# multi-template-matching/MultiTemplateMatching-Python

Hardware: AMD Instinct MI355X
Metric: Mpixel-correlations/s (higher is better)
Workload: dtype u8

## Files before the change

include/mtm_hip.h:

```cpp
#ifndef MTM_HIP_H
#define MTM_HIP_H

#include <stddef.h>
#include <stdint.h>

#ifdef __cplusplus
extern "C" {
#endif

#define MTM_ABI_VERSION 9

#define MTM_U8  0
#define MTM_F32 1
#define MTM_U16 2

#define MTM_TM_SQDIFF        0
#define MTM_TM_SQDIFF_NORMED 1
#define MTM_TM_CCORR         2
#define MTM_TM_CCORR_NORMED  3
#define MTM_TM_CCOEFF        4
#define MTM_TM_CCOEFF_NORMED 5

#define MTM_PEAKS_LOCAL  0
#define MTM_PEAKS_GLOBAL 1
// ... 5 lines not shown
#define MTM_KERNEL_NAIVE 1
#define MTM_KERNEL_DOT4  2
#define MTM_KERNEL_MFMA  3
#define MTM_KERNEL_MFMA16 4

#define MTM_KERNEL_MFMA_F32 5

#define MTM_OPT_KERNEL      1
#define MTM_OPT_PEAK_BORDER 2
#define MTM_OPT_HIT_CAPACITY 3
#define MTM_OPT_DOT4_VARIANT 4
#define MTM_OPT_EXACT_DIV 5
#define MTM_OPT_HITS_ONLY 6
#define MTM_OPT_F32_MFMA 7
#define MTM_OPT_BATCH_MAX_ROWS 8
#define MTM_OPT_BOXES_MAX_FLOATS 9

#define MTM_OK            0
#define MTM_E_INVALID    -1
#define MTM_E_HIP        -2
#define MTM_E_NO_DEVICE  -3
#define MTM_E_STATE      -4
#define MTM_E_OVERFLOW   -5
#define MTM_E_COMM       -6

typedef struct mtm_ctx mtm_ctx;

typedef struct mtm_templ {
    const void* px;
    const void* mask;
    int32_t rows, cols, chans, dtype;
    int64_t row_stride;
    int64_t mask_row_stride;
} mtm_templ;

typedef struct mtm_hit {
    int32_t templ_idx;
    int32_t x, y, w, h;
    float   score;
} mtm_hit;

typedef struct mtm_box_unit {
    int32_t templ_idx;
    int32_t y0, x0, rows, cols;
} mtm_box_unit;

typedef struct mtm_point {
    int32_t templ_idx, x, y;
} mtm_point;

typedef struct mtm_timing {
    float total_ms;
    float score_ms;
    float peaks_ms;
    float ncc_kernel_ms;
    int32_t ncc_launches;
    int32_t kernel_used;
    int64_t n_hits;
    int32_t hits_only;
    float   sclk_mhz;
    float   ncc_sum_ms;
    int32_t f32_route;
    int32_t sq_launches;
    float   masked_stat_ms;
    int32_t f32_pieces;
} mtm_timing;

int         mtm_abi_version(void);
int         mtm_device_count(void);
const char* mtm_last_error(void);
int         mtm_ctx_create(mtm_ctx** out, int device_id);
void        mtm_ctx_destroy(mtm_ctx* ctx);
int         mtm_set_option(mtm_ctx* ctx, int option, int64_t value);
int         mtm_get_option(mtm_ctx* ctx, int option, int64_t* value);
#define MTM_POISON_SCRATCH 1
#define MTM_POISON_LDS     2
#define MTM_POISON_ARENAS  4
int         mtm_debug_poison(mtm_ctx* ctx, int pattern_byte, int what);
int         mtm_debug_quotient_check(mtm_ctx* ctx, uint64_t n_cases, uint64_t seed, uint64_t* out4);
int         mtm_debug_tail_split(int h, int w, double thr);
int         mtm_debug_templ_stats(const void* px, int rows, int cols, int chans, int dtype, int method, double* out7);
#define MTM_CLASS_TILING_FIELDS 12
int         mtm_debug_class_tilings(mtm_ctx* ctx, int32_t* out, int cap_classes);
int         mtm_debug_device_nms(mtm_ctx* ctx, const mtm_hit* hits, int64_t n, int rows, int cols, int max_side,
                                 double score_threshold, int ascending, double max_overlap, int64_t n_min, int64_t n_max,
                                 mtm_hit* out, int64_t capacity, int64_t* n_champions, int64_t* n_undecided);
#define MTM_PEAK_SCAN           0
#define MTM_PEAK_SCAN_BATCH     1
#define MTM_PEAK_SEGMENTS       2
#define MTM_PEAK_VERIFY_MAPS    3
#define MTM_PEAK_VERIFY_HASH    4
#define MTM_PEAK_EXTREMUM       5
#define MTM_PEAK_EXTREMUM_BATCH 6
typedef struct mtm_peak_pass {
    int32_t        n_maps, route, mode_min, border;
    float          thr, thr_q;
    int32_t        img_rows, holes, pattern_byte, reserved;
    int64_t        hit_cap;
    const int32_t* dims;
    const float*   maps;
    const uint8_t* flags;
    const mtm_hit* cands;
    int64_t        n_cands, cand_count, cand_cap;
    mtm_hit*       records;
    int64_t        capacity;
    uint64_t*      count;
    int32_t*       raw;
    int32_t*       trivial;
    int64_t        n_ints;
    uint64_t*      keys;
    mtm_hit*       ext_hits;
    uint64_t*      list_counts;
    int64_t        list_cap;
    int64_t*       info;
} mtm_peak_pass;
int         mtm_debug_peak_pass(mtm_ctx* ctx, const mtm_peak_pass* args);
#define MTM_STATS_FORMS 2
typedef struct mtm_window_stats {
    int32_t        rows, cols, h, w, num_type, form;
    int32_t        tail_s, sb0, sb1, lay_r0, lay_r1, pattern_byte, zero_header, reserved;
    const uint8_t* image;
    double*        t0;
    double*        sum2;
    double*        sq;
    double*        rsq;
    double*        blk;
    double*        blkq;
    uint8_t*       u8;
    uint8_t*       u8b;
    uint64_t*      header;
    int64_t*       info;
} mtm_window_stats;
int         mtm_debug_window_stats(mtm_ctx* ctx, const mtm_window_stats* args);
void*       mtm_host_alloc(size_t bytes);
void        mtm_host_free(void* p);

int mtm_set_image(mtm_ctx* ctx, const void* px, int rows, int cols, int chans, int dtype,
                  int64_t row_stride_bytes);
int mtm_set_image_downscaled(mtm_ctx* ctx, const void* px, int rows, int cols, int chans, int dtype,
                             int64_t row_stride_bytes, int factor);

int mtm_set_templates(mtm_ctx* ctx, const mtm_templ* templs, int n_templ, int method);

typedef struct mtm_variant {
    int32_t rot90;
    int32_t flip_lr;
    int32_t flip_ud;
    int32_t rows, cols;
    int32_t down;
} mtm_variant;
int mtm_set_templates_augmented(mtm_ctx* ctx, const mtm_templ* bases, int n_bases,
                                const mtm_variant* variants, int n_variants, int method);

int mtm_score_map(mtm_ctx* ctx, int templ_idx, float* out, int64_t out_row_stride_bytes);

int mtm_find_matches(mtm_ctx* ctx, int mode, double score_threshold,
                     mtm_hit* out, int64_t capacity, int64_t* n_out);

int mtm_find_matches_image(mtm_ctx* ctx, const void* px, int rows, int cols, int chans, int dtype,
                           int64_t row_stride_bytes, int mode, double score_threshold,
                           mtm_hit* out, int64_t capacity, int64_t* n_out);

int mtm_find_matches_image_nms(mtm_ctx* ctx, const void* px, int rows, int cols, int chans, int dtype,
                               int64_t row_stride_bytes, double score_threshold, double max_overlap, int64_t n_object,
                               mtm_hit* out, int64_t capacity, int64_t* n_out);

// ... 114 lines not shown
```

multitemplatematching-python_amd/MTM/_lib.py:

```python
import ctypes
import struct
import os
import threading
import weakref

import numpy as np

_HERE = os.path.dirname(os.path.abspath(__file__))
LIB_PATH = os.environ.get("MTM_LIB_PATH") or os.path.join(_HERE, "libmtm_hip.so")

MTM_U8, MTM_F32, MTM_U16 = 0, 1, 2
GROUP_EXCHANGE_HOST, GROUP_EXCHANGE_RCCL = 0, 1
PEAKS_LOCAL, PEAKS_GLOBAL = 0, 1
BORDER_CONSTANT, BORDER_NEAREST = 0, 1
KERNEL_AUTO, KERNEL_NAIVE, KERNEL_DOT4, KERNEL_MFMA = 0, 1, 2, 3
OPT_KERNEL, OPT_PEAK_BORDER, OPT_HIT_CAPACITY, OPT_DOT4_VARIANT, OPT_EXACT_DIV, OPT_HITS_ONLY, OPT_F32_MFMA = 1, 2, 3, 4, 5, 6, 7
OPT_BATCH_MAX_ROWS = 8
OPT_BOXES_MAX_FLOATS = 9
ALL_OPTIONS = (OPT_KERNEL, OPT_PEAK_BORDER, OPT_HIT_CAPACITY, OPT_DOT4_VARIANT, OPT_EXACT_DIV, OPT_HITS_ONLY, OPT_F32_MFMA,
               OPT_BATCH_MAX_ROWS, OPT_BOXES_MAX_FLOATS)
BATCH_MAX_ROWS = 65535
POISON_SCRATCH, POISON_LDS, POISON_ARENAS = 1, 2, 4
E_OVERFLOW = -5
E_HIP = -2
COMM_ID_BYTES = 128
ABI_VERSION = 9


class MtmTempl(ctypes.Structure):
    _fields_ = [("px", ctypes.c_void_p), ("mask", ctypes.c_void_p),
                ("rows", ctypes.c_int32), ("cols", ctypes.c_int32),
                ("chans", ctypes.c_int32), ("dtype", ctypes.c_int32),
                ("row_stride", ctypes.c_int64), ("mask_row_stride", ctypes.c_int64)]


class MtmHit(ctypes.Structure):
    _fields_ = [("templ_idx", ctypes.c_int32), ("x", ctypes.c_int32), ("y", ctypes.c_int32),
                ("w", ctypes.c_int32), ("h", ctypes.c_int32), ("score", ctypes.c_float)]


class MtmTiming(ctypes.Structure):
    _fields_ = [("total_ms", ctypes.c_float), ("score_ms", ctypes.c_float),
                ("peaks_ms", ctypes.c_float), ("ncc_kernel_ms", ctypes.c_float),
                ("ncc_launches", ctypes.c_int32), ("kernel_used", ctypes.c_int32),
                ("n_hits", ctypes.c_int64), ("hits_only", ctypes.c_int32), ("sclk_mhz", ctypes.c_float),
                ("ncc_sum_ms", ctypes.c_float), ("f32_route", ctypes.c_int32),
                ("sq_launches", ctypes.c_int32), ("masked_stat_ms", ctypes.c_float),
                ("f32_pieces", ctypes.c_int32)]


HIT_DTYPE = np.dtype([("templ_idx", "<i4"), ("x", "<i4"), ("y", "<i4"), ("w", "<i4"), ("h", "<i4"),
                      ("score", "<f4")])
BOX_UNIT_DTYPE = np.dtype([("templ_idx", "<i4"), ("y0", "<i4"), ("x0", "<i4"), ("rows", "<i4"), ("cols", "<i4")])
BLOCK_DTYPE = np.dtype([("x", "<i4"), ("y", "<i4"), ("w", "<i4"), ("h", "<i4")])
POINT_DTYPE = np.dtype([("templ_idx", "<i4"), ("x", "<i4"), ("y", "<i4")])
assert HIT_DTYPE.itemsize == ctypes.sizeof(MtmHit) == 24
TEMPL_DTYPE = np.dtype([("px", "<u8"), ("mask", "<u8"), ("rows", "<i4"), ("cols", "<i4"), ("chans", "<i4"),
                        ("dtype", "<i4"), ("row_stride", "<i8"), ("mask_row_stride", "<i8")])
assert TEMPL_DTYPE.itemsize == ctypes.sizeof(MtmTempl) == 48
VARIANT_DTYPE = np.dtype([("rot90", "<i4"), ("flip_lr", "<i4"), ("flip_ud", "<i4"), ("rows", "<i4"), ("cols", "<i4"),
                          ("down", "<i4")])

PEAK_SCAN, PEAK_SCAN_BATCH, PEAK_SEGMENTS, PEAK_VERIFY_MAPS, PEAK_VERIFY_HASH, PEAK_EXTREMUM, PEAK_EXTREMUM_BATCH = range(7)
PEAK_INFO_FIELDS = ("grid_x", "grid_y", "grid_z", "list_cap", "n_lists", "verify_blocks", "hash_slots", "extremum_blocks")


class MtmPeakPass(ctypes.Structure):
    _fields_ = [("n_maps", ctypes.c_int32), ("route", ctypes.c_int32), ("mode_min", ctypes.c_int32), ("border", ctypes.c_int32),
                ("thr", ctypes.c_float), ("thr_q", ctypes.c_float),
                ("img_rows", ctypes.c_int32), ("holes", ctypes.c_int32), ("pattern_byte", ctypes.c_int32), ("reserved", ctypes.c_int32),
                ("hit_cap", ctypes.c_int64),
                ("dims", ctypes.c_void_p), ("maps", ctypes.c_void_p), ("flags", ctypes.c_void_p), ("cands", ctypes.c_void_p),
                ("n_cands", ctypes.c_int64), ("cand_count", ctypes.c_int64), ("cand_cap", ctypes.c_int64),
                ("records", ctypes.c_void_p), ("capacity", ctypes.c_int64), ("count", ctypes.c_void_p),
                ("raw", ctypes.c_void_p), ("trivial", ctypes.c_void_p), ("n_ints", ctypes.c_int64),
                ("keys", ctypes.c_void_p), ("ext_hits", ctypes.c_void_p), ("list_counts", ctypes.c_void_p),
                ("list_cap", ctypes.c_int64), ("info", ctypes.c_void_p)]


STATS_FORMS = (8, 4)
STATS_INFO_FIELDS = ("st_pitch", "blk_pitch", "pitch", "form", "grid_x", "grid_y", "n_cus", "kernel_ns")


class MtmWindowStats(ctypes.Structure):
    _fields_ = [("rows", ctypes.c_int32), ("cols", ctypes.c_int32), ("h", ctypes.c_int32), ("w", ctypes.c_int32),
                ("num_type", ctypes.c_int32), ("form", ctypes.c_int32),
                ("tail_s", ctypes.c_int32), ("sb0", ctypes.c_int32), ("sb1", ctypes.c_int32), ("lay_r0", ctypes.c_int32),
                ("lay_r1", ctypes.c_int32), ("pattern_byte", ctypes.c_int32), ("zero_header", ctypes.c_int32),
                ("reserved", ctypes.c_int32),
                ("image", ctypes.c_void_p), ("t0", ctypes.c_void_p), ("sum2", ctypes.c_void_p), ("sq", ctypes.c_void_p),
                ("rsq", ctypes.c_void_p), ("blk", ctypes.c_void_p), ("blkq", ctypes.c_void_p), ("u8", ctypes.c_void_p),
                ("u8b", ctypes.c_void_p), ("header", ctypes.c_void_p), ("info", ctypes.c_void_p)]


_P = ctypes.POINTER
SYMBOLS = {
    "mtm_abi_version": (ctypes.c_int, []),
    "mtm_device_count": (ctypes.c_int, []),
    "mtm_last_error": (ctypes.c_char_p, []),
    "mtm_ctx_create": (ctypes.c_int, [_P(ctypes.c_void_p), ctypes.c_int]),
    "mtm_ctx_destroy": (None, [ctypes.c_void_p]),
    "mtm_set_option": (ctypes.c_int, [ctypes.c_void_p, ctypes.c_int, ctypes.c_int64]),
    "mtm_get_option": (ctypes.c_int, [ctypes.c_void_p, ctypes.c_int, _P(ctypes.c_int64)]),
    "mtm_debug_poison": (ctypes.c_int, [ctypes.c_void_p, ctypes.c_int, ctypes.c_int]),
    "mtm_debug_quotient_check": (ctypes.c_int, [ctypes.c_void_p, ctypes.c_uint64, ctypes.c_uint64, _P(ctypes.c_uint64)]),
    "mtm_debug_tail_split": (ctypes.c_int, [ctypes.c_int, ctypes.c_int, ctypes.c_double]),
    "mtm_debug_class_tilings": (ctypes.c_int, [ctypes.c_void_p, _P(ctypes.c_int32), ctypes.c_int]),
    "mtm_debug_templ_stats": (ctypes.c_int, [ctypes.c_void_p, ctypes.c_int, ctypes.c_int, ctypes.c_int, ctypes.c_int,
                                             ctypes.c_int, _P(ctypes.c_double)]),
    "mtm_debug_device_nms": (ctypes.c_int, [ctypes.c_void_p, ctypes.c_void_p, ctypes.c_int64, ctypes.c_int, ctypes.c_int,
                                            ctypes.c_int, ctypes.c_double, ctypes.c_int, ctypes.c_double, ctypes.c_int64,
                                            ctypes.c_int64, ctypes.c_void_p, ctypes.c_int64, _P(ctypes.c_int64),
                                            _P(ctypes.c_int64)]),
    "mtm_debug_peak_pass": (ctypes.c_int, [ctypes.c_void_p, ctypes.c_void_p]),
    "mtm_debug_window_stats": (ctypes.c_int, [ctypes.c_void_p, ctypes.c_void_p]),
    "mtm_set_image": (ctypes.c_int, [ctypes.c_void_p, ctypes.c_void_p, ctypes.c_int, ctypes.c_int,
                                     ctypes.c_int, ctypes.c_int, ctypes.c_int64]),
    "mtm_set_image_downscaled": (ctypes.c_int, [ctypes.c_void_p, ctypes.c_void_p, ctypes.c_int, ctypes.c_int, ctypes.c_int,
                                                ctypes.c_int, ctypes.c_int64, ctypes.c_int]),
    "mtm_set_templates": (ctypes.c_int, [ctypes.c_void_p, ctypes.c_void_p, ctypes.c_int, ctypes.c_int]),
    "mtm_set_templates_augmented": (ctypes.c_int, [ctypes.c_void_p, ctypes.c_void_p, ctypes.c_int, ctypes.c_void_p, ctypes.c_int,
                                                   ctypes.c_int]),
    "mtm_score_map": (ctypes.c_int, [ctypes.c_void_p, ctypes.c_int, ctypes.c_void_p, ctypes.c_int64]),
    "mtm_find_matches": (ctypes.c_int, [ctypes.c_void_p, ctypes.c_int, ctypes.c_double, ctypes.c_void_p,
                                        ctypes.c_int64, _P(ctypes.c_int64)]),
    "mtm_find_matches_image": (ctypes.c_int, [ctypes.c_void_p, ctypes.c_void_p, ctypes.c_int, ctypes.c_int, ctypes.c_int,
                                              ctypes.c_int, ctypes.c_int64, ctypes.c_int, ctypes.c_double, ctypes.c_void_p,
                                              ctypes.c_int64, _P(ctypes.c_int64)]),
    "mtm_find_matches_image_nms": (ctypes.c_int, [ctypes.c_void_p, ctypes.c_void_p, ctypes.c_int, ctypes.c_int, ctypes.c_int,
                                                  ctypes.c_int, ctypes.c_int64, ctypes.c_double, ctypes.c_double, ctypes.c_int64,
                                                  ctypes.c_void_p, ctypes.c_int64, _P(ctypes.c_int64)]),
    "mtm_find_matches_image_sharded_nms": (ctypes.c_int, [ctypes.c_void_p, ctypes.c_void_p, ctypes.c_int, ctypes.c_int, ctypes.c_int,
                                                          ctypes.c_int, ctypes.c_int64, ctypes.c_double, ctypes.c_double,
                                                          ctypes.c_int64, ctypes.c_int, ctypes.c_void_p, ctypes.c_int,
                                                          ctypes.c_void_p, ctypes.c_int64, _P(ctypes.c_int64)]),
    "mtm_find_matches_batch": (ctypes.c_int, [ctypes.c_void_p, ctypes.c_void_p, ctypes.c_int, ctypes.c_int, ctypes.c_int,
                                              ctypes.c_int, ctypes.c_int, ctypes.c_int64, ctypes.c_int, ctypes.c_double,
                                              ctypes.c_void_p, ctypes.c_int64, ctypes.c_void_p, _P(ctypes.c_int64)]),
    "mtm_find_matches_pyramid": (ctypes.c_int, [ctypes.c_void_p, ctypes.c_void_p, ctypes.c_int, ctypes.c_int, ctypes.c_int,
                                                ctypes.c_int, ctypes.c_int64, ctypes.c_int, ctypes.c_int, ctypes.c_double,
                                                ctypes.c_double, ctypes.c_int, ctypes.c_int, ctypes.c_void_p, ctypes.c_int64,
                                                _P(ctypes.c_int64)]),
    "mtm_find_matches_boxes": (ctypes.c_int, [ctypes.c_void_p, ctypes.c_void_p, ctypes.c_int, ctypes.c_int, ctypes.c_int,
                                              ctypes.c_int, ctypes.c_int64, ctypes.c_void_p, ctypes.c_int, ctypes.c_int,
                                              ctypes.c_double, ctypes.c_void_p, ctypes.c_int64, ctypes.c_void_p,
                                              _P(ctypes.c_int64)]),
    "mtm_track_boxes": (ctypes.c_int, [ctypes.c_void_p, ctypes.c_void_p, ctypes.c_int, ctypes.c_int, ctypes.c_int,
                                       ctypes.c_int, ctypes.c_int, ctypes.c_int64, ctypes.c_void_p, ctypes.c_int, ctypes.c_int,
                                       ctypes.c_int, ctypes.c_double, ctypes.c_void_p]),
    "mtm_track_boxes_nbhd": (ctypes.c_int, [ctypes.c_void_p, ctypes.c_void_p, ctypes.c_int, ctypes.c_int, ctypes.c_int,
                                            ctypes.c_int, ctypes.c_int, ctypes.c_int64, ctypes.c_void_p, ctypes.c_int,
                                            ctypes.c_int, ctypes.c_int, ctypes.c_double, ctypes.c_void_p, ctypes.c_void_p]),
    "mtm_track_boxes_adapt": (ctypes.c_int, [ctypes.c_void_p, ctypes.c_void_p, ctypes.c_int, ctypes.c_int, ctypes.c_int,
                                             ctypes.c_int, ctypes.c_int, ctypes.c_int64, ctypes.c_void_p, ctypes.c_int,
                                             ctypes.c_int, ctypes.c_int, ctypes.c_double, ctypes.c_void_p, ctypes.c_void_p,
                                             ctypes.c_int, ctypes.c_void_p, ctypes.c_void_p]),
    "mtm_track_boxes_reacquire": (ctypes.c_int, [ctypes.c_void_p, ctypes.c_void_p, ctypes.c_int, ctypes.c_int, ctypes.c_int,
                                                 ctypes.c_int, ctypes.c_int, ctypes.c_int64, ctypes.c_void_p, ctypes.c_int,
                                                 ctypes.c_int, ctypes.c_int, ctypes.c_double, ctypes.c_void_p,
                                                 ctypes.c_void_p, ctypes.c_int, ctypes.c_void_p, ctypes.c_void_p]),
    "mtm_track_boxes_sets": (ctypes.c_int, [ctypes.c_void_p, ctypes.c_void_p, ctypes.c_int, ctypes.c_int, ctypes.c_int,
                                            ctypes.c_int, ctypes.c_int, ctypes.c_int64, ctypes.c_void_p, ctypes.c_int,
                                            ctypes.c_void_p, ctypes.c_void_p, ctypes.c_int, ctypes.c_int, ctypes.c_double,
                                            ctypes.c_int, ctypes.c_void_p, ctypes.c_void_p]),
    "mtm_match_blocks": (ctypes.c_int, [ctypes.c_void_p, ctypes.c_void_p, ctypes.c_int64, ctypes.c_void_p, ctypes.c_int64,
                                        ctypes.c_int, ctypes.c_int, ctypes.c_int, ctypes.c_int, ctypes.c_void_p, ctypes.c_int,
                                        ctypes.c_int, ctypes.c_int, ctypes.c_void_p, ctypes.c_void_p]),
    "mtm_debug_plan_blocks": (ctypes.c_int, [ctypes.c_int, ctypes.c_int, ctypes.c_int, ctypes.c_int, ctypes.c_void_p,
                                             ctypes.c_int, ctypes.c_int, ctypes.c_int64, ctypes.c_void_p, ctypes.c_int64,
                                             _P(ctypes.c_int64), ctypes.c_void_p, ctypes.c_void_p, ctypes.c_void_p]),
    "mtm_hit_neighbourhoods": (ctypes.c_int, [ctypes.c_void_p, ctypes.c_void_p, ctypes.c_int, ctypes.c_int, ctypes.c_int,
                                              ctypes.c_int, ctypes.c_int64, ctypes.c_void_p, ctypes.c_int, ctypes.c_void_p]),
    "mtm_find_matches_next": (ctypes.c_int, [ctypes.c_void_p, ctypes.c_int, ctypes.c_double, ctypes.c_void_p,
                                             ctypes.c_int64, _P(ctypes.c_int64), ctypes.c_void_p, ctypes.c_int,
                                             ctypes.c_int, ctypes.c_int, ctypes.c_int, ctypes.c_int64]),
    "mtm_find_matches_async": (ctypes.c_int, [ctypes.c_void_p, ctypes.c_int, ctypes.c_double]),
    "mtm_find_matches_wait": (ctypes.c_int, [ctypes.c_void_p, ctypes.c_void_p, ctypes.c_int64, ctypes.POINTER(ctypes.c_int64)]),
    "mtm_last_hits": (ctypes.c_int, [ctypes.c_void_p, ctypes.c_void_p, ctypes.c_int64, _P(ctypes.c_int64)]),
    "mtm_last_score_map": (ctypes.c_int, [ctypes.c_void_p, ctypes.c_int, ctypes.c_void_p, ctypes.c_int64]),
    "mtm_get_timing": (ctypes.c_int, [ctypes.c_void_p, _P(MtmTiming)]),
    "mtm_nms": (ctypes.c_int, [ctypes.c_void_p, ctypes.c_int64, ctypes.c_double, ctypes.c_int,
                               ctypes.c_int64, ctypes.c_double, ctypes.c_void_p, _P(ctypes.c_int64)]),
    "mtm_nms_segments": (ctypes.c_int, [ctypes.c_void_p, ctypes.c_void_p, ctypes.c_int64, ctypes.c_double, ctypes.c_int,
                                        ctypes.c_double, ctypes.c_void_p, ctypes.c_void_p]),
    "mtm_group_create": (ctypes.c_int, [_P(ctypes.c_void_p), _P(ctypes.c_int), ctypes.c_int]),
    "mtm_group_destroy": (None, [ctypes.c_void_p]),
    "mtm_group_size": (ctypes.c_int, [ctypes.c_void_p]),
    "mtm_group_ctx": (ctypes.c_void_p, [ctypes.c_void_p, ctypes.c_int]),
    "mtm_group_set_option": (ctypes.c_int, [ctypes.c_void_p, ctypes.c_int, ctypes.c_int64]),
    "mtm_group_shards": (ctypes.c_int, [ctypes.c_void_p, ctypes.c_void_p, ctypes.c_int, ctypes.c_int, ctypes.c_int,
# ... 222 lines not shown
    n = len(blocks)
    code = _DT_CODES[np.dtype(dtype)]
    n_tiles = ctypes.c_int64(0)
    chunk_of = np.zeros(n, dtype=np.int32)
    toff = np.zeros(n, dtype=np.int64)
    maps = np.zeros((n, 4), dtype=np.int32)
    args = (int(shape[0]), int(shape[1]), int(chans), code, blocks.ctypes.data, n, int(margin), int(budget_bytes))
    check(lib.mtm_debug_plan_blocks(*args, None, 0, ctypes.byref(n_tiles), chunk_of.ctypes.data, toff.ctypes.data,
                                    maps.ctypes.data), "mtm_debug_plan_blocks")
    tiles = np.zeros((n_tiles.value, 3), dtype=np.int32)
    check(lib.mtm_debug_plan_blocks(*args, tiles.ctypes.data, n_tiles.value, ctypes.byref(n_tiles), None, None, None),
          "mtm_debug_plan_blocks")
    return tiles, chunk_of, toff, maps


def debug_templ_stats(template, method):
    a = np.ascontiguousarray(template)
    chans = 1 if a.ndim == 2 else a.shape[2]
    out = (ctypes.c_double * len(TEMPL_STATS_FIELDS))()
    check(load().mtm_debug_templ_stats(a.ctypes.data, a.shape[0], a.shape[1], chans, _dtype_code(a), int(method), out),
          "mtm_debug_templ_stats")
    return np.array(out[:], dtype=np.float64)


class Context(_RecordMemo):

    def __init__(self, device=None):
        lib = load()
        if device is None:
            device = int(os.environ.get("MTM_DEVICE", os.environ.get("LOCAL_RANK", "0")))
            n = lib.mtm_device_count()
            if n > 0:
                device %= n
        h = ctypes.c_void_p()
        check(lib.mtm_ctx_create(ctypes.byref(h), int(device)), "mtm_ctx_create")
        self._lib = lib
        self._h = h
        self.device = device
        self.lock = threading.RLock()
        self._keep = []
        self._rec_key, self._rec, self._rec_keep = None, None, None
        _LIVE.add(self)
        k = os.environ.get("MTM_KERNEL")
        if k:
            self.set_option(OPT_KERNEL, {"auto": 0, "naive": 1, "dot4": 2, "mfma": 3}[k.lower()])
        b = os.environ.get("MTM_PEAK_BORDER")
        if b:
            self.set_option(OPT_PEAK_BORDER, {"constant": 0, "nearest": 1}[b.lower()])

    def close(self):
        _LIVE.discard(self)
        if self._h:
            self._lib.mtm_ctx_destroy(self._h)
            self._h = None

    def __del__(self):
        try:
            self.close()
        except Exception:
            pass

    def set_option(self, opt, value):
        check(self._lib.mtm_set_option(self._h, int(opt), int(value)), "mtm_set_option")

    def get_option(self, opt):
        v = ctypes.c_int64(0)
        check(self._lib.mtm_get_option(self._h, int(opt), ctypes.byref(v)), "mtm_get_option")
        return int(v.value)

    def options(self):
        return {o: self.get_option(o) for o in ALL_OPTIONS}

    def debug_poison(self, pattern=0xFF, what=7):
        check(self._lib.mtm_debug_poison(self._h, int(pattern), int(what)), "mtm_debug_poison")

    def class_tilings(self):
        nf = len(CLASS_TILING_FIELDS)
        n = self._lib.mtm_debug_class_tilings(self._h, None, 0)
        check(min(n, 0), "mtm_debug_class_tilings")
        buf = (ctypes.c_int32 * (nf * max(n, 1)))()
        check(min(self._lib.mtm_debug_class_tilings(self._h, buf, n), 0), "mtm_debug_class_tilings")
        return [dict(zip(CLASS_TILING_FIELDS, buf[k * nf:(k + 1) * nf])) for k in range(n)]

    def debug_quotient_check(self, n_cases=1 << 28, seed=1):
        out = (ctypes.c_uint64 * 4)()
        check(self._lib.mtm_debug_quotient_check(self._h, int(n_cases), int(seed), out), "mtm_debug_quotient_check")
        return {"cases": int(out[0]), "mismatches": int(out[1]), "took_division": int(out[2]), "max_ulp_distance": int(out[3])}

    def debug_device_nms(self, hits, rows, cols, max_side, score_threshold, max_overlap, ascending=False, n_min=0,
                         n_max=1 << 18, out=None):
        hits = np.ascontiguousarray(hits, dtype=HIT_DTYPE)
        n = len(hits)
        if out is None:
            out = np.empty(max(n, 1), dtype=HIT_DTYPE)
        assert out.dtype == HIT_DTYPE and out.flags.c_contiguous
        nc, nu = ctypes.c_int64(0), ctypes.c_int64(0)
        check(self._lib.mtm_debug_device_nms(self._h, hits.ctypes.data, n, int(rows), int(cols), int(max_side),
                                             float(score_threshold), int(bool(ascending)), float(max_overlap), int(n_min),
                                             int(n_max), out.ctypes.data, len(out), ctypes.byref(nc), ctypes.byref(nu)),
              "mtm_debug_device_nms")
        return out[:nc.value], out[nc.value:nc.value + nu.value]

    def debug_peak_pass(self, maps, route, thr, mode_min=False, border=BORDER_NEAREST, hit_cap=4096, templ_hw=None, img_rows=0,
                        flags=None, holes=False, cands=None, cand_count=None, cand_cap=None, thr_q=None, pattern=0xFF,
                        records=None):
        maps = [np.ascontiguousarray(m, dtype=np.float32) for m in maps]
        n = len(maps)
        assert n >= 1 and all(m.ndim == 2 for m in maps)
        templ_hw = [(1, 1)] * n if templ_hw is None else list(templ_hw)
        dims = np.array([[m.shape[0], m.shape[1], hw[0], hw[1]] for m, hw in zip(maps, templ_hw)], dtype=np.int32)
        packed = np.concatenate([m.ravel() for m in maps])
        batch = route in (PEAK_SCAN_BATCH, PEAK_EXTREMUM_BATCH)
        n_img = (int(dims[0, 0]) + int(dims[0, 2]) - 1) // int(img_rows) if batch and img_rows > 0 else 1
        n_ints = n * max(n_img, 1)
        max_oh, max_ow = int(dims[:, 0].max()), int(dims[:, 1].max())
        n_sx = (max_ow + 255) // 256
        a = MtmPeakPass()
        a.n_maps, a.route, a.mode_min, a.border = n, int(route), int(bool(mode_min)), int(border)
        a.thr = float(thr)
        a.thr_q = float(thr_q) if thr_q is not None else float(np.float32(-np.float32(thr)) if mode_min else np.float32(thr))
        a.img_rows, a.holes, a.pattern_byte, a.hit_cap = int(img_rows), int(bool(holes)), int(pattern), int(hit_cap)
        a.dims, a.maps = dims.ctypes.data, packed.ctypes.data
        if flags is not None:
            flags = np.ascontiguousarray(flags, dtype=np.uint8)
            assert flags.shape == (n, max_oh, n_sx), (flags.shape, (n, max_oh, n_sx))
            a.flags = flags.ctypes.data
        if cands is not None:
            cands = np.ascontiguousarray(cands, dtype=HIT_DTYPE)
            a.cands = cands.ctypes.data if len(cands) else None
            a.n_cands = len(cands)
            a.cand_count = len(cands) if cand_count is None else int(cand_count)
            a.cand_cap = max(len(cands), 1) if cand_cap is None else int(cand_cap)
        if records is None:
            records = np.zeros(int(hit_cap), dtype=HIT_DTYPE)
        assert records.dtype == HIT_DTYPE and records.flags.c_contiguous and records.flags.writeable
        count = np.zeros(1, dtype=np.uint64)
        raw, trivial = np.zeros(n_ints, dtype=np.int32), np.zeros(n_ints, dtype=np.int32)
        keys, ext_hits = np.zeros(2 * n_ints, dtype=np.uint64), np.zeros(2 * n_ints, dtype=HIT_DTYPE)
        list_counts = np.zeros(n * n_sx, dtype=np.uint64)
        info = np.zeros(8, dtype=np.int64)
        a.records, a.capacity, a.count = records.ctypes.data, len(records), count.ctypes.data
        a.raw, a.trivial, a.n_ints = raw.ctypes.data, trivial.ctypes.data, n_ints
        a.keys, a.ext_hits = keys.ctypes.data, ext_hits.ctypes.data
        a.list_counts, a.list_cap, a.info = list_counts.ctypes.data, len(list_counts), info.ctypes.data
        check(self._lib.mtm_debug_peak_pass(self._h, ctypes.byref(a)), "mtm_debug_peak_pass")
        shape = (n_img, n) if batch else (n,)
        return {"records": records, "count": int(count[0]), "raw": raw.reshape(shape), "trivial": trivial.reshape(shape),
                "keys": keys.reshape(shape + (2,)), "ext_hits": ext_hits.reshape(shape + (2,)), "list_counts": list_counts,
                "info": dict(zip(PEAK_INFO_FIELDS, (int(v) for v in info)))}

    def debug_window_stats(self, image, h, w, num_type, form=0, planes=("t0", "sum2", "sq", "rsq", "blk"), tail_s=0, units=None,
                           convert_rows=None, zero_header=True, pattern=0xA5):
        image = np.ascontiguousarray(image, dtype=np.uint8)
        assert image.ndim == 2
        rows, cols = image.shape
        oh, ow = rows - h + 1, cols - w + 1
        st_pitch = (ow + 3) // 4 * 4
        blk_pitch = (st_pitch + 15) // 16
        pitch = (cols + 512 + 63) // 64 * 64
        a = MtmWindowStats()
        a.rows, a.cols, a.h, a.w, a.num_type, a.form = rows, cols, int(h), int(w), int(num_type), int(form)
        a.tail_s, a.pattern_byte, a.zero_header = int(tail_s), int(pattern), int(bool(zero_header))
        a.sb0, a.sb1 = (0, -1) if units is None else (int(units[0]), int(units[1]))
        a.lay_r0, a.lay_r1 = (0, 0) if convert_rows is None else (int(convert_rows[0]), int(convert_rows[1]))
        a.image = image.ctypes.data
        out = {}
# ... 443 lines not shown
```

multitemplatematching-python_amd/csrc/mtm_context.hip:

```cpp
#include <cstdio>
#include "mtm_ctx.h"

using namespace mtm;
using namespace mtmi;
#include "mtm_k_image.hip.h"

namespace mtmi {

int prepare_slot(mtm_ctx* c, mtm_ctx::ImageSlot& sl, int src_rows, int src_cols, int chans, int dtype, hipStream_t stream,
                 int factor, SlotGeom* g) {
    (void)c;
    const size_t esz = elem_size(dtype);
    const size_t tight = (size_t)src_cols * chans * esz;
    MTMC(sl.raw.ensure(tight * src_rows));
    const int rows = src_rows / factor, cols = src_cols / factor;
    const int rows_alloc = rows + kPadRows;
    const int pitch = (int)round_up((size_t)cols + kPadCols, 64);
    const size_t f32_bytes = sizeof(float) * pitch * rows_alloc * chans;
    const size_t u8_bytes = (size_t)pitch * rows_alloc * chans;
    const long long geom = (((long long)rows * 65536 + cols) * 8 + chans) * 4 + dtype;
    const size_t caps[3] = {sl.f32.cap, sl.u8.cap, sl.u8b.cap};
    MTMC(sl.f32.ensure(f32_bytes));
    const bool u16_planes = dtype == MTM_U16 && chans == 1;
    const size_t u8b_bytes = u16_planes ? 2 * u8_bytes : u8_bytes;
// ... 209 lines not shown
    int lo = 0, hi = 0;
    (void)hipDeviceGetStreamPriorityRange(&lo, &hi);
    HIPC(hipStreamCreateWithPriority(&c->copy_stream, hipStreamNonBlocking, hi));
    return MTM_OK;
}

}

extern "C" {

int mtm_device_count(void) {
    int n = 0;
    if (hipGetDeviceCount(&n) != hipSuccess) return 0;
    return n;
}

void* mtm_host_alloc(size_t bytes) {
    void* p = nullptr;
    const hipError_t e = hipHostMalloc(&p, bytes ? bytes : 1, hipHostMallocPortable | hipHostMallocMapped);
    if (e != hipSuccess) {
        set_error(std::string("mtm_host_alloc: ") + hipGetErrorString(e));
        return nullptr;
    }
    return p;
}

void mtm_host_free(void* p) {
    if (p) (void)hipHostFree(p);
}

int mtm_ctx_create(mtm_ctx** out, int device_id) {
    if (!out) {
        set_error("mtm_ctx_create: null output");
        return MTM_E_INVALID;
    }
    int n = 0;
    if (hipGetDeviceCount(&n) != hipSuccess || n <= 0) {
        set_error("no HIP device visible (libmtm_hip has no CPU fallback)");
        return MTM_E_NO_DEVICE;
    }
    if (device_id < 0 || device_id >= n) {
        set_error("device id out of range");
        return MTM_E_INVALID;
    }
    HIPC(hipSetDevice(device_id));
    mtm_ctx* c = new mtm_ctx();
    c->device = device_id;
    hipError_t e = hipStreamCreateWithFlags(&c->stream, hipStreamNonBlocking);
    for (int i = 0; i < 4 && e == hipSuccess; ++i) e = hipEventCreate(&c->ev[i]);
    if (e != hipSuccess) {
        set_error(std::string("context creation: ") + hipGetErrorString(e));
        delete c;
        return MTM_E_HIP;
    }
    if (const char* v = std::getenv("MTM_UPLOAD_BANDS")) {
        std::vector<double> f;
        for (const char* q = v; *q;) {
            char* end = nullptr;
            const double x = std::strtod(q, &end);
            if (end == q) break;
            if (x > 0.0 && x <= 1.0 && (f.empty() || x > f.back())) f.push_back(x);
            q = *end == ',' ? end + 1 : end;
        }
        if (!f.empty()) {
            f.back() = 1.0;
            c->upload_bands = f;
        }
    }
    if (const char* v = std::getenv("MTM_CAND_PINNED")) c->cand_pinned = std::atoi(v);
    if (const char* v = std::getenv("MTM_FUSE_LAYOUT")) c->fuse_layout = std::atoi(v);
    if (const char* v = std::getenv("MTM_SEG_SKIP")) c->seg_skip = std::atoi(v);
    if (const char* v = std::getenv("MTM_BAND_MIN_FILL")) c->band_min_fill = std::atof(v);
    if (const char* v = std::getenv("MTM_TEMPL_ON_DEVICE")) c->templ_on_device = std::atoi(v);
    if (const char* v = std::getenv("MTM_ROW_MUX")) c->row_mux = std::atoi(v);
    if (const char* v = std::getenv("MTM_FUSE_STATS")) c->fuse_stats = std::atoi(v);
    if (const char* v = std::getenv("MTM_MFMA_R2")) c->mfma_r2 = std::atoi(v) != 0;
    if (const char* v = std::getenv("MTM_F32_MFMA")) c->f32_mfma = std::atoi(v);
    if (const char* v = std::getenv("MTM_MASKSQ_FUSED")) c->masksq_fused = std::atoi(v);
    if (const char* v = std::getenv("MTM_SPARSE_MAPS")) c->sparse_maps = std::atoi(v);
    if (const char* v = std::getenv("MTM_NMS_DEVICE_MIN")) c->nms_device_min = std::atoll(v) < 0 ? (1ll << 60) : std::max(1, std::atoi(v));
    if (const char* v = std::getenv("MTM_SCREEN_L1")) c->screen_l1 = std::atoi(v);
    if (const char* v = std::getenv("MTM_TAIL_SCREEN")) c->tail_screen = std::atoi(v) != 0;
    if (const char* v = std::getenv("MTM_TAIL_SPLIT")) c->tail_split_force = std::max(0, std::atoi(v));
    if (const char* v = std::getenv("MTM_HOST_TRACE")) c->host_trace = std::atoi(v) != 0;
    if (const char* v = std::getenv("MTM_CLASS_LANES")) c->class_lanes = std::max(1, std::min(8, std::atoi(v)));
    if (const char* v = std::getenv("MTM_COMM_TIMEOUT_S")) c->comm_timeout_s = std::atof(v);
    if (const char* v = std::getenv("MTM_HITS_ONLY")) c->hits_only = std::atoi(v);
    if (const char* v = std::getenv("MTM_EXACT_DIV")) c->exact_div = std::atoi(v);
    {
        hipDeviceProp_t prop;
        if (hipGetDeviceProperties(&prop, c->device) == hipSuccess) c->n_cus = prop.multiProcessorCount;
    }
    if (ensure_copy_stream(c) != MTM_OK) c->copy_stream = nullptr;
    if (c->class_lanes > 1) (void)ensure_lanes(c, 1);
    *out = c;
    return MTM_OK;
}

void mtm_ctx_destroy(mtm_ctx* c) {
    if (!c) return;
    if (c->host_trace) {
        static const char* kPhase[24] = {"entry", "args checked", "templates placed", "call set up", "band 0 copy queued",
                                         "band 0 layout + statistics queued", "band 0 score queued", "last band copy queued",
                                         "last band score queued", "score pass queued", "stream synchronised", "hits verified",
                                         "hits sorted", "(banded: image slot prepared)", "(banded: before the first copy call)", "return",
                                         "(banded: score pass entered)", "(banded: copy stream ready)", "(fm_begin: decisions taken)", "", "", "", "", ""};
        for (int k = 0; k < 24; ++k)
            if (c->trace_n[k] > 0)
                std::fprintf(stderr, "[mtm host trace] %-36s %9.1f us after entry (mean of %lld)\n", kPhase[k],
                             c->trace_acc[k] / (double)c->trace_n[k], c->trace_n[k]);
    }
    (void)hipSetDevice(c->device);
    mtm_comm_destroy(c);
    (void)hipStreamSynchronize(c->stream);
    if (c->copy_stream) (void)hipStreamSynchronize(c->copy_stream);
    if (c->pyr_sub) mtm_ctx_destroy(c->pyr_sub);
    for (DevBuf* b : {&c->win_tpx, &c->win_toff, &c->win_buf, &c->win_hits, &c->win_flags, &c->pyr_wins, &c->box_td,
                      &c->box_units, &c->box_tiles, &c->trk_units, &c->trk_tiles, &c->trk_keys, &c->trk_out,
                      &c->trk_nbhd, &c->trk_tpx, &c->trk_toff, &c->trk_td, &c->trk_pass, &c->trk_lost, &c->trk_sets,
                      &c->blk_tpx, &c->blk_toff, &c->blk_td, &c->blk_blocks, &c->blk_units, &c->blk_tiles, &c->blk_keys,
                      &c->blk_nbhd})
        b->release();
    for (auto& sl : c->slot)
        for (DevBuf* b : {&sl.raw, &sl.u8, &sl.u8b, &sl.f32}) b->release();
    for (DevBuf* b : {&c->tsrc, &c->usrc_dev, &c->tsums_dev, &c->tgather, &c->slab_raw, &c->seg_flags, &c->hits_t, &c->nms_buf, &c->nms_dbg, &c->peak_dbg, &c->stats_dbg, &c->td_u, &c->td_v,
                      &c->mbf_maps, &c->f32_sq, &c->mbf_stats, &c->mbf_mu, &c->mbf_list, &c->mbf_best}) b->release();
    for (DevBuf* b : {&c->td, &c->tlist, &c->weights, &c->packs, &c->apacks, &c->maps, &c->hs1, &c->hs2, &c->stats, &c->hits,
                      &c->counters, &c->sched, &c->cands, &c->mask_td, &c->chash, &c->raw16, &c->stats_hi, &c->tsum, &c->stats_rsq, &c->stats_blk, &c->sq_planes, &c->comm_send,
                      &c->comm_recv})
        b->release();
    if (c->pinned) (void)hipHostFree(c->pinned);
    if (c->pin_small) (void)hipHostFree(c->pin_small);
    if (c->comm_pin) (void)hipHostFree(c->comm_pin);
    if (c->next_ready) (void)hipEventDestroy(c->next_ready);
    for (hipEvent_t e : c->band_ev) (void)hipEventDestroy(e);
    if (c->lane_fork) (void)hipEventDestroy(c->lane_fork);
    if (c->f32_built) (void)hipEventDestroy(c->f32_built);
    for (auto& L : c->lanes) {
        if (L.stream) {
            (void)hipStreamSynchronize(L.stream);
            (void)hipStreamDestroy(L.stream);
        }
        if (L.done) (void)hipEventDestroy(L.done);
        if (L.slab_fork) (void)hipEventDestroy(L.slab_fork);
        for (hipEvent_t e : L.slab_done) (void)hipEventDestroy(e);
        for (hipStream_t s2 : L.slab_streams) {
            (void)hipStreamSynchronize(s2);
            (void)hipStreamDestroy(s2);
        }
        for (DevBuf* b : {&L.stats, &L.stats_rsq, &L.stats_blk, &L.hs1, &L.hs2, &L.raw16, &L.slab_raw, &L.stats_hi, &L.mask_td, &L.sched})
            b->release();
    }
    if (c->slab_fork) (void)hipEventDestroy(c->slab_fork);
    for (hipEvent_t e : c->slab_done) (void)hipEventDestroy(e);
    for (hipStream_t s2 : c->slab_streams) {
        (void)hipStreamSynchronize(s2);
        (void)hipStreamDestroy(s2);
    }
    if (c->copy_stream) (void)hipStreamDestroy(c->copy_stream);
    for (auto* evs : {&c->ncc_ev, &c->sq_ev})
        for (auto& p : *evs) {
            (void)hipEventDestroy(p.first);
            (void)hipEventDestroy(p.second);
        }
    for (int i = 0; i < 4; ++i)
        if (c->ev[i]) (void)hipEventDestroy(c->ev[i]);
    if (c->stream) (void)hipStreamDestroy(c->stream);
    delete c;
}

int mtm_set_option(mtm_ctx* c, int option, int64_t value) {
    if (!c) return MTM_E_INVALID;
    MTM_NOT_IN_FLIGHT(c, "mtm_set_option");
    switch (option) {
        case MTM_OPT_KERNEL:
            if (value < MTM_KERNEL_AUTO || value > MTM_KERNEL_MFMA) break;
            if (c->opt_kernel != (int)value) c->placed = false;
            c->opt_kernel = (int)value;
            return MTM_OK;
        case MTM_OPT_PEAK_BORDER:
            if (value != MTM_BORDER_CONSTANT && value != MTM_BORDER_NEAREST) break;
            c->opt_border = (int)value;
            return MTM_OK;
        case MTM_OPT_HIT_CAPACITY:
            if (value < 1) break;
            c->hit_cap = value;
            return MTM_OK;
        case MTM_OPT_EXACT_DIV:
            c->exact_div = value < 0 ? 0 : value > 2 ? 2 : (int)value;
            return MTM_OK;
        case MTM_OPT_HITS_ONLY:
            c->hits_only = value ? 1 : 0;
            c->fuse_backoff = 0;
            c->backoff_len = 16;
            c->np1_backoff = 0;
            c->np1_backoff_len = 16;
            return MTM_OK;
        case MTM_OPT_F32_MFMA:
            if (value < 0 || value > 4) break;
            if ((c->f32_mfma != 0) != (value != 0)) c->placed = false;
            c->f32_mfma = (int)value;
            c->np1_backoff = 0;
            c->np1_backoff_len = 16;
            return MTM_OK;
        case MTM_OPT_DOT4_VARIANT:
            if (!dot_variant_ok(value)) break;
            c->dot_variant = (int)value;
            return MTM_OK;
        case MTM_OPT_BATCH_MAX_ROWS:
            if (value < 1 || value > kBatchMaxRows) break;
            c->batch_max_rows = (int)value;
            return MTM_OK;
// ... 25 lines not shown
    return MTM_E_INVALID;
}

__global__ __launch_bounds__(256) void poison_scratch_kernel(uint32_t pat, int sleeps, uint32_t* sink) {
    uint32_t buf[160];
    volatile uint32_t* vb = buf;
    for (int i = 0; i < 160; ++i) vb[i] = pat;
    for (int i = 0; i < sleeps; ++i) __builtin_amdgcn_s_sleep(127);
    uint32_t acc = 0;
    for (int i = 0; i < 160; ++i) acc += vb[(i * 7 + (int)threadIdx.x) % 160] != pat;
    if (acc) atomicAdd(sink, acc);
}
constexpr int kPoisonLdsBytes = 40 * 1024;
__global__ __launch_bounds__(256) void poison_lds_kernel(uint32_t pat, int sleeps, uint32_t* sink) {
    __shared__ uint32_t lds[kPoisonLdsBytes / 4];
    for (int i = threadIdx.x; i < kPoisonLdsBytes / 4; i += 256) lds[i] = pat;
    __syncthreads();
    for (int i = 0; i < sleeps; ++i) __builtin_amdgcn_s_sleep(127);
    if (lds[(threadIdx.x * 13) % (kPoisonLdsBytes / 4)] != pat) atomicAdd(sink, 1u);
}

int mtm_debug_poison(mtm_ctx* c, int pattern_byte, int what) {
    if (!c) return MTM_E_INVALID;
    MTM_NOT_IN_FLIGHT(c, "mtm_debug_poison");
    HIPC(hipSetDevice(c->device));
    const uint32_t b = (uint32_t)(pattern_byte & 0xFF), pat = b | (b << 8) | (b << 16) | (b << 24);
    if (c->n_cus == 0) {
        hipDeviceProp_t prop;
        HIPC(hipGetDeviceProperties(&prop, c->device));
        c->n_cus = prop.multiProcessorCount;
    }
    MTMC(c->sched.ensure(sizeof(unsigned int) * (1 + 4096 + 8 * 32)));
    uint32_t* sink = c->sched.as<uint32_t>() + 4096;
    if (what & MTM_POISON_SCRATCH)
        hipLaunchKernelGGL(poison_scratch_kernel, dim3(c->n_cus * 8 * 3), dim3(256), 0, c->stream, pat, 4, sink);
    if (what & MTM_POISON_LDS)
        hipLaunchKernelGGL(poison_lds_kernel, dim3(c->n_cus * 4 * 3), dim3(256), 0, c->stream, pat, 4, sink);
    if (what & MTM_POISON_ARENAS) {
        auto fill = [&](mtm_ctx::DevBuf& d) -> int {
            if (d.p && d.cap) HIPC(hipMemsetAsync(d.p, (int)b, d.cap, c->stream));
            return MTM_OK;
        };
        for (mtm_ctx::DevBuf* d : {&c->stats, &c->stats_rsq, &c->stats_blk, &c->hs1, &c->hs2, &c->raw16, &c->slab_raw,
                                   &c->stats_hi, &c->maps, &c->sq_planes, &c->mbf_maps, &c->f32_sq, &c->mbf_stats, &c->mbf_mu,
                                   &c->trk_units, &c->trk_keys, &c->trk_out, &c->trk_nbhd, &c->trk_tpx, &c->trk_toff, &c->trk_td,
                                   &c->trk_pass, &c->trk_lost, &c->trk_sets, &c->blk_tpx, &c->blk_toff, &c->blk_td, &c->blk_blocks, &c->blk_units,
                                   &c->blk_tiles, &c->blk_keys, &c->blk_nbhd, &c->sub_pts, &c->sub_out, &c->nms_buf, &c->peak_dbg, &c->stats_dbg})
            MTMC(fill(*d));
        for (auto& ln : c->lanes)
            for (mtm_ctx::DevBuf* d : {&ln.stats, &ln.stats_rsq, &ln.stats_blk, &ln.hs1, &ln.hs2, &ln.raw16, &ln.slab_raw, &ln.stats_hi})
                MTMC(fill(*d));
        c->maps_valid = false;
        c->sq_valid = false;
        c->f32_sq_valid = false;
    }
    HIPC(hipStreamSynchronize(c->stream));
    HIPC(hipGetLastError());
    return MTM_OK;
}

int mtm_debug_class_tilings(mtm_ctx* c, int32_t* out, int cap_classes) {
    if (!c || (!out && cap_classes > 0)) return MTM_E_INVALID;
    MTM_NOT_IN_FLIGHT(c, "mtm_debug_class_tilings");
    if (!c->placed) {
        set_error("mtm_debug_class_tilings: no template set is placed (run a search first)");
        return MTM_E_STATE;
    }
    const int n = (int)c->classes.size();
    for (int k = 0; k < n && k < cap_classes; ++k) {
        const mtm_ctx::SizeClass& sc = c->classes[(size_t)k];
        int32_t* r = out + (size_t)k * MTM_CLASS_TILING_FIELDS;
        r[0] = sc.h;
        r[1] = sc.w;
        r[2] = (int32_t)sc.members.size();
        r[3] = sc.kernel;
        r[4] = sc.rm_nt;
        r[5] = sc.rm_R;
        r[6] = sc.kp_nseg;
        r[7] = sc.r2;
        r[8] = sc.tail_ok ? 1 : 0;
        r[9] = (size_t)k < c->tail_last.size() ? c->tail_last[(size_t)k] : 0;
        r[10] = (int32_t)sc.slabs.size();
        r[11] = sc.slab_nt;
    }
    return n;
}

__device__ __forceinline__ uint64_t dq_mix(uint64_t z) {
    z += 0x9E3779B97F4A7C15ull;
    z = (z ^ (z >> 30)) * 0xBF58476D1CE4E5B9ull;
    z = (z ^ (z >> 27)) * 0x94D049BB133111EBull;
    return z ^ (z >> 31);
}
__global__ __launch_bounds__(256) void quotient_check_kernel(uint64_t n_per_thread, uint64_t seed, unsigned long long* out) {
    const uint64_t gid = (uint64_t)blockIdx.x * blockDim.x + threadIdx.x;
    unsigned long long bad = 0, div = 0, far = 0;
    for (uint64_t k = 0; k < n_per_thread; ++k) {
        const uint64_t idx = gid * n_per_thread + k;
        const uint64_t r0 = dq_mix(seed ^ (idx * 4u)), r1 = dq_mix(seed ^ (idx * 4u + 1u)), r2 = dq_mix(seed ^ (idx * 4u + 2u)),
                       r3 = dq_mix(seed ^ (idx * 4u + 3u));
        const double e_w = (double)(1ull + (r0 >> (20 + (r3 & 31)))), e_t = (double)(1ull + (r1 >> (20 + ((r3 >> 5) & 31))));
        const double sq = sqrt(e_w), tn = sqrt(e_t);
        const double tt = sq * tn;
        const double rr = (1.0 / sq) * (1.0 / tn);
        double num;
        if ((idx & 1u) == 0u) {
            const double u = (double)(int64_t)(r2 >> 11) * 0x1p-52 - 1.0;
            num = u * tt * 1.2;
            if (r3 & (1ull << 40)) num = rint(num);
        } else {
            uint32_t fb = 0x35800000u + (uint32_t)(r2 % (0x3f800000u - 0x35800000u));
            if ((idx & 7u) == 7u) fb = 0x00000001u + (uint32_t)(r2 % 0x02000000u);
            const double lo_f = (double)__uint_as_float(fb), hi_f = (double)__uint_as_float(fb + 1u);
            const double mid = 0.5 * (lo_f + hi_f);
            num = mid * tt;
            const int step = (int)((r3 >> 44) % 9u) - 4;
            num = __longlong_as_double(__double_as_longlong(num) + (long long)step);
            if (r3 & (1ull << 41)) num = -num;
        }
        const double q0 = num * rr;
        const double qr = num / tt;
        const float ref = (float)qr;
        const float got = quotient_as_float(num, tt, rr);
        bad += __float_as_uint(ref) != __float_as_uint(got);
        if ((idx & 7u) != 7u) bad += __float_as_uint(ref) != __float_as_uint(quotient_as_float<false>(num, tt, rr));
        div += quotient_needs_division(q0);
        if (fabs(qr) > 0x1p-1000 && fabs(qr) < 0x1p1000) {
            const long long d = __double_as_longlong(fabs(q0)) - __double_as_longlong(fabs(qr));
            const unsigned long long ad = (unsigned long long)(d < 0 ? -d : d);
            far = ad > far ? ad : far;
        }
    }
    atomicAdd(&out[1], bad);
    atomicAdd(&out[2], div);
    atomicMax(&out[3], far);
}

int mtm_debug_quotient_check(mtm_ctx* c, uint64_t n_cases, uint64_t seed, uint64_t* out4) {
    if (!c || !out4) return MTM_E_INVALID;
    MTM_NOT_IN_FLIGHT(c, "mtm_debug_quotient_check");
    HIPC(hipSetDevice(c->device));
    const int blocks = 2048, threads = 256;
    const uint64_t per = (n_cases + (uint64_t)blocks * threads - 1) / ((uint64_t)blocks * threads);
    MTMC(c->sched.ensure(sizeof(unsigned int) * (1 + 4096 + 8 * 32)));
    unsigned long long* acc = reinterpret_cast<unsigned long long*>(c->sched.as<uint32_t>() + 4096 + 16);
    HIPC(hipMemsetAsync(acc, 0, 4 * sizeof(unsigned long long), c->stream));
    hipLaunchKernelGGL(quotient_check_kernel, dim3(blocks), dim3(threads), 0, c->stream, per, seed, acc);
    unsigned long long h[4] = {0, 0, 0, 0};
    HIPC(hipMemcpyAsync(h, acc, sizeof(h), hipMemcpyDeviceToHost, c->stream));
    HIPC(hipStreamSynchronize(c->stream));
    HIPC(hipGetLastError());
    out4[0] = per * (uint64_t)blocks * threads;
    out4[1] = h[1];
    out4[2] = h[2];
    out4[3] = h[3];
    return MTM_OK;
}

int mtm_set_image_downscaled(mtm_ctx* c, const void* px, int rows, int cols, int chans, int dtype,
                             int64_t row_stride_bytes, int factor) {
    if (!c) {
        set_error("mtm_set_image: null context");
        return MTM_E_INVALID;
    }
    MTM_NOT_IN_FLIGHT(c, "mtm_set_image");
    MTMC(check_image_args(px, rows, cols, chans, dtype, row_stride_bytes, "mtm_set_image"));
// ... 18 lines not shown
```

multitemplatematching-python_amd/csrc/mtm_ctx.h:

```cpp
#pragma once
#include <hip/hip_runtime.h>

#include <algorithm>
#include <chrono>
#include <cmath>
#include <cstdlib>
#include <cstring>
#include <functional>
#include <map>
#include <string>
#include <thread>
#include <tuple>
#include <vector>

#include "mtm_kernels.h"
#include "mtm_mfma_params.h"
#include "mtm_bf16_params.h"
#include "mtm_score_params.h"
#include "mtm_templates_params.h"
#include "mtm_internal.h"
#include "mtm_route.h"
#include "mtm_peak_sizing.h"

struct ncclComm;
// ... 18 lines not shown
    } while (0)
#define MTM_NOT_IN_FLIGHT(c, who)                                                                         \
    do {                                                                                                  \
        if ((c)->fm_in_flight) {                                                                          \
            set_error(std::string(who) + ": a mtm_find_matches_async call is in flight (collect it with " \
                      "mtm_find_matches_wait first)");                                                    \
            return MTM_E_INVALID;                                                                         \
        }                                                                                                 \
    } while (0)


inline size_t round_up(size_t v, size_t a) { return (v + a - 1) / a * a; }

constexpr int kBatchMaxRows = 65535;
constexpr double kBatchChunkBytes = 8.0 * (1ull << 30);

inline size_t elem_size(int dtype) { return dtype == MTM_U8 ? 1 : dtype == MTM_U16 ? 2 : 4; }

struct DevBuf {
    void* p = nullptr;
    size_t cap = 0;
    int ensure(size_t bytes) {
        if (bytes <= cap) return MTM_OK;
        const size_t want = round_up(bytes + bytes / 8, 256);
        void* fresh = nullptr;
        HIPC(hipMalloc(&fresh, want));
        if (p) (void)hipFree(p);
        p = fresh;
        cap = want;
        return MTM_OK;
    }
    void release() {
        if (p) (void)hipFree(p);
        p = nullptr;
        cap = 0;
    }
    template <typename T> T* as() const { return reinterpret_cast<T*>(p); }
};

struct HostTempl {
    int rows = 0, cols = 0, chans = 0, dtype = 0;
    bool masked = false;
    std::vector<double> px;
    std::vector<double> mask;
    TemplStats st;
    int cls = -1;
    bool on_device = false;
    UnitSrc src{};
    double sum_t = 0.0;
    double mask_ones = 0.0;
    unsigned long long mask_key = 0;
};

struct SizeClass {
    int h = 0, w = 0;
    bool masked = false;
    bool all_u8 = true;
    bool all_u16 = true;
    bool all_f32 = true;
    int kernel = MTM_KERNEL_AUTO;
    int rm_nt = 0, rm_R = 0;
    int kp_nseg = 0;
    struct Slab {
        int r0, r1, c0, c1, ch;
        long long apack_off;
        int tlist_off;
    };
    std::vector<Slab> slabs;
    int slab_nt = 0, slab_R = 0;
    int r2 = 0;
    bool tail_ok = false;
    int tail_split = 0;
    long long mask_rm_off = -1;
    double mask_ones = 0.0;
    int n_pad = 0;
    long long tsum_off = -1;
    std::vector<int> members;
    int tlist_off = 0;
    bool masked_int = false;
    unsigned long long mask_hash = 0;
    long long mask_pack_off = -1;
    bool mask_bf16 = false;
    long long mbf_off_u = -1, mbf_off_v = -1, mbf_group_bytes = 0;
    long long apack_off = 0;
    long long group_bytes = 0;
};

}

struct mtm_ctx {
    using DevBuf = mtmi::DevBuf;
    using HostTempl = mtmi::HostTempl;
    using SizeClass = mtmi::SizeClass;
    using CallRoute = mtmi::CallRoute;
    using TemplDev = mtm::TemplDev;
    using UnitSrc = mtm::UnitSrc;
    int device = 0;
    hipStream_t stream = nullptr;
    hipEvent_t ev[4] = {nullptr, nullptr, nullptr, nullptr};
    std::vector<std::pair<hipEvent_t, hipEvent_t>> ncc_ev;
    std::vector<std::pair<hipEvent_t, hipEvent_t>> sq_ev;
    int cand_pinned = 1;
    int fuse_layout = 1;
    int lay_r0 = 0, lay_r1 = 0;
    int masksq_fused = 1;

    bool have_image = false;
    int rows = 0, cols = 0, chans = 0, dtype = 0;
    int u8_pitch = 0, f32_pitch = 0, rows_alloc = 0;
    struct ImageSlot {
        DevBuf raw, u8, u8b, f32;
        long long geom = -1;
        bool f32_valid = true;
    } slot[2];
    int cur = 0;
    DevBuf sq_planes;
    bool sq_valid = false;
    hipStream_t copy_stream = nullptr;
    long long nms_device_min = 4096;
    DevBuf nms_buf;
    DevBuf nms_dbg;
    DevBuf peak_dbg;
    DevBuf stats_dbg;
    int sparse_maps = 1;
    DevBuf seg_flags, hits_t;
    hipEvent_t next_ready = nullptr;
    hipStream_t stats_stream = nullptr;
    int screen_l1 = 1;
    int tail_screen = 1;
    int tail_split_force = 0;
    std::vector<int> tail_valid;
    std::vector<int> tail_last;
    int f32_mfma = 1;
    int np1_backoff = 0, np1_backoff_len = 16;
    int seg_skip = 1;
    int templ_on_device = 1;
    int mfma_r2 = 1;
    struct Lane {
        DevBuf stats, stats_rsq, stats_blk, hs1, hs2, raw16, slab_raw, stats_hi, mask_td, sched;
        hipStream_t stream = nullptr;
        hipEvent_t done = nullptr;
        std::vector<hipStream_t> slab_streams;
        std::vector<hipEvent_t> slab_done;
        hipEvent_t slab_fork = nullptr;
    };
    std::vector<Lane> lanes;
    bool slab_fork_early = false;
    hipEvent_t lane_fork = nullptr;
    hipEvent_t f32_built = nullptr;
    int class_lanes = 2;
    std::vector<hipStream_t> slab_streams;
    std::vector<hipEvent_t> slab_done;
    hipEvent_t slab_fork = nullptr;
    std::vector<hipEvent_t> band_ev;
    int banded_cls = -1;
    std::vector<double> upload_bands{0.25, 1.0};
    bool host_trace = false;
    double trace_acc[24] = {0};
    long long trace_n[24] = {0};
    long long trace_calls = 0;
    double trace_t0 = 0.0;

    bool have_templ = false;
    bool placed = false;
    int method = MTM_TM_CCOEFF_NORMED;
    std::vector<HostTempl> templs;
    std::vector<SizeClass> classes;
    std::vector<TemplDev> td_host;
    std::vector<int> tlist_host;
    std::vector<int> list2d;
    int list2d_off = 0;
    size_t maps_floats = 0;
    std::vector<UnitSrc> usrc_host;
    size_t usrc_units = 0;
    std::vector<uint8_t> tstage;
    bool stage_pending = false;
    bool place_pending = false;
    DevBuf slab_raw;
    DevBuf td_u, td_v, mbf_maps, f32_sq, mbf_stats, mbf_mu, mbf_list, mbf_best;
    bool f32_sq_valid = false;
    DevBuf tsrc, usrc_dev, tsums_dev, tgather;
    DevBuf td, tlist, weights, packs, apacks, maps, hs1, hs2, stats, hits, counters, sched, cands, mask_td, chash, raw16, stats_hi, tsum, stats_rsq, stats_blk;

    int opt_kernel = MTM_KERNEL_AUTO;
    int opt_border = MTM_BORDER_NEAREST;
    int64_t hit_cap = 1 << 18;
    int dot_variant = 0;
    int fuse_stats = 1;
    int row_mux = 1;
    double band_min_fill = 1.0;
    int n_cus = 0;
    int hits_only = 1;
    int backoff_len = 16;
    int fuse_backoff = 0;
    bool maps_valid = false;
    CallRoute fm;
    bool fm_in_flight = false;
    const void* cands_zeroed = nullptr;
    int exact_div = 1;
    int auto_kernel = MTM_KERNEL_MFMA;
    int batch_max_rows = mtmi::kBatchMaxRows;

    mtm_timing timing{};
    std::vector<mtm_hit> last_hits;
    void* pin_small = nullptr;
    void* pinned = nullptr;
    size_t pinned_cap = 0;
    void* comm_pin = nullptr;
    size_t comm_pin_cap = 0;
    std::vector<uint8_t> templ_blob;
    uint64_t templ_gen = 0;
    uint64_t win_gen = 0;
    std::vector<uint8_t> win_blob;
    DevBuf win_tpx, win_toff, win_buf, win_hits, win_flags;
    mtm_ctx* pyr_sub = nullptr;
// ... 50 lines not shown
    d.u8_pitch = c->u8_pitch;
    d.f32_pitch = c->f32_pitch;
    d.u8_plane = (long long)c->u8_pitch * c->rows_alloc;
    d.f32_plane = (long long)c->f32_pitch * c->rows_alloc;
    return d;
}

constexpr int kMfmaMaxW = 256;
inline long long mfma_group_bytes(int h, int w, int chans) { return (long long)chans * h * ((w + 63) / 64) * 1024; }
inline int kp_blocks(int rows, int nseg) { return (rows * nseg + 3) / 4; }
inline int mfma_groups_alloc(int n) { return (((n + 15) / 16) + 1) & ~1; }
inline long long rm_pack_bytes(int h, int w, int R) { return (long long)(h + 3 * R - 1) * ((w + 63) / 64) * 1024; }
inline long long class_rm_pack_bytes(const SizeClass& sc) {
    return sc.kp_nseg ? 2LL * kp_blocks(sc.h + 2 * sc.rm_R - 1, sc.kp_nseg) * 1024 : rm_pack_bytes(sc.h, sc.w, sc.rm_R);
}
inline int bf16_nkb(int w) { return (w + 31) / 32; }
inline long long bf16_group_bytes(int h, int w, int chans) { return (long long)chans * h * bf16_nkb(w) * 1024; }
inline int mfma_lds_pitch(int nb) { return (16 + 4 * nb + 1) * 16; }
inline int rm_tile_rows(int h, int R) { return std::min(h + 2 * R - 1, kMfChunkH) + (kMfRows - 1) * 2 * R; }
inline int rm_group_templates(int n, int h, int w) {
    int nt = 1;
    while (nt < n) nt <<= 1;
    const size_t lds_pitch = (size_t)mfma_lds_pitch((w + 63) / 64);
    while (nt < 16 && (size_t)rm_tile_rows(h, 16 / nt) * lds_pitch > 72 * 1024) nt <<= 1;
    return nt;
}
constexpr int64_t kCandListMax = 4096LL * 256;
inline unsigned long long cand_list_cap(const mtm_ctx* c) { return (unsigned long long)std::min<int64_t>(c->hit_cap, kCandListMax); }

struct ImageArgs {
    const void* px;
    int rows, cols, chans, dtype;
    int64_t stride;
};
struct SlotGeom {
    int rows, cols, rows_alloc, pitch;
    size_t u8_bytes;
};

inline bool f32_refined(const mtm_ctx* c) { return c->f32_mfma == 1 || c->f32_mfma == 3; }
inline float bf16_rig_eps(int chans, int h, int nkb, int np = 3) {
    if (np == 1) return (float)(0.0078125 * 1.002 + 2.0 * (2.0 * 1.0 * (double)chans * h * nkb * 5.97e-8));
    return (float)(2.0 * (3.0518e-5 + 2.0 * 3.0 * (double)chans * h * nkb * 5.97e-8));
}
inline float bf16_ext_eps(int chans, int h, int nkb, int np = 3) {
    if (np == 1) return bf16_rig_eps(chans, h, nkb, 1);
    return (float)(3.0518e-5 + 3.0 * (double)chans * h * nkb * 5.97e-8);
}

int prepare_slot(mtm_ctx* c, mtm_ctx::ImageSlot& sl, int src_rows, int src_cols, int chans, int dtype, hipStream_t stream,
                 int factor, SlotGeom* out);
int upload_rows_u8c1(mtm_ctx::ImageSlot& sl, const SlotGeom& g, const void* src, int64_t src_stride, int r0, int r1,
                     hipStream_t stream, bool skip_f32, hipEvent_t copy_done = nullptr, hipEvent_t before_kernels = nullptr,
                     bool convert = true);
int upload_rows_u16c1(mtm_ctx::ImageSlot& sl, const SlotGeom& g, const void* src, int64_t src_stride, int r0, int r1,
                      hipStream_t stream, hipEvent_t copy_done = nullptr, hipEvent_t before_kernels = nullptr);
int upload_image(mtm_ctx* c, mtm_ctx::ImageSlot& sl, const void* src, int64_t src_stride, int src_rows, int src_cols,
                 int chans, int dtype, hipStream_t stream, int factor = 1);
int upload_image_stack(mtm_ctx* c, mtm_ctx::ImageSlot& sl, const void* const* px, int n, int64_t src_stride, int rows,
                       int cols, int chans, int dtype, hipStream_t stream);
int upload_image_pair(mtm_ctx* c, mtm_ctx::ImageSlot& sl, const void* px0, int64_t stride0, const void* px1, int64_t stride1,
                      int rows, int cols, int chans, int dtype, hipStream_t stream);
void adopt_image(mtm_ctx* c, int rows, int cols, int chans, int dtype);
int parse_templ_blob(const std::vector<uint8_t>& b, std::vector<BlobTempl>& out, const char* who, bool u16_ok);
int prepare_window_templates(mtm_ctx* c, const std::vector<BlobTempl>& tl);
int prepare_box_td(mtm_ctx* c, const std::vector<BlobTempl>& tl);
using WindowPeakLaunch = std::function<int(mtm_hit* hits, unsigned long long cap, unsigned long long* counter,
                                           unsigned long long* best, int* nontrivial)>;
int window_peak_pass(mtm_ctx* c, int n, bool global, const WindowPeakLaunch& launch, std::vector<unsigned long long>& best,
                     std::vector<mtm_hit>& recs, const char* who);
int derive_downscaled_u8(mtm_ctx* dst, const mtm_ctx::ImageSlot& src, int src_rows, int src_cols, int chans, int factor,
                         hipStream_t stream);
int check_image_args(const void* px, int rows, int cols, int chans, int dtype, int64_t row_stride_bytes, const char* who);
int ensure_f32_plane(mtm_ctx* c);
int upload_rows_f32c1(mtm_ctx::ImageSlot& sl, const SlotGeom& g, const void* src, int64_t src_stride, int r0, int r1, hipStream_t stream);
int ensure_copy_stream(mtm_ctx* c);
int ensure_lanes(mtm_ctx* c, int n);
int comm_allgather_hits_flagged(mtm_ctx* c, const mtm_hit* local, int64_t n_local, int32_t my_flag, mtm_hit* out,
                                int64_t capacity, int64_t* counts_out, int64_t* n_out, std::vector<int32_t>* flags_out);
int place_templates(mtm_ctx* c);
bool dot_variant_ok(int64_t v);
int launch_stats(mtm_ctx* c, CallRoute& R, const SizeClass& sc, StatPlanes* out, int sb0 = 0, int sb1 = -1);
int launch_tail_consts(mtm_ctx* c, const SizeClass& sc, int split, hipStream_t stream);
int launch_ncc(mtm_ctx* c, CallRoute& R, const SizeClass& sc, int list_off, int n_list, const StatPlanes& st, int only_li = -1,
               int yb0 = 0, int yb1 = -1);
int ensure_maps(mtm_ctx* c);
int run_score_all(mtm_ctx* c, CallRoute& R);
bool banded_ok(mtm_ctx* c, const ImageArgs& a, bool* single_band);
int run_score_banded(mtm_ctx* c, CallRoute& R, const ImageArgs& a);
int collect_ncc_time(mtm_ctx* c);

}
```

multitemplatematching-python_amd/csrc/mtm_launch.hip:

```cpp
#include "mtm_ctx.h"

using namespace mtm;
using namespace mtmi;
#include "mtm_k_stats.hip.h"
#include "mtm_k_score.hip.h"
#include "mtm_refine.hip.h"
#include "mtm_maskf32.hip.h"

namespace {

struct DotVariant {
    int px, py, nt;
    bool wide;
    void (*fn)(DotParams, const TemplDev*, const int*, const uint8_t*, StatPlanes, float*);
};
#define DOTV(PX, PY, NT, W) {PX, PY, NT, W, ncc_dot4_kernel<PX, PY, NT, W>}
const DotVariant kDotVariants[] = {
    DOTV(4, 4, 4, false),
    DOTV(4, 4, 2, false),
    DOTV(8, 2, 4, false),
    DOTV(8, 4, 2, false),
    DOTV(4, 2, 4, false),
    DOTV(8, 2, 2, false),
    DOTV(4, 2, 8, false),
// ... 5 lines not shown
MfmaFn mfma_raw_fn(bool row_mux, bool packed_k) {
    MfmaSel s;
    s.method = kMfRaw;
    s.rm = row_mux;
    s.kp = packed_k;
    return mfma_kernel(s);
}

dim3 work_grid(int n_work) { return dim3((unsigned)(((n_work + 7) / 8) * 8)); }

int event_pair(std::vector<std::pair<hipEvent_t, hipEvent_t>>& evs, int i, std::pair<hipEvent_t, hipEvent_t>** out) {
    if ((int)evs.size() <= i) {
        hipEvent_t a, b;
        HIPC(hipEventCreate(&a));
        HIPC(hipEventCreate(&b));
        evs.emplace_back(a, b);
    }
    *out = &evs[(size_t)i];
    return MTM_OK;
}

MfmaParams mfma_geometry(const uint8_t* img, const ImageDev& d, int chans, int h, int w, int oh, int ow, int method) {
    MfmaParams p{};
    p.img = img;
    p.pitch = d.u8_pitch;
    p.plane = d.u8_plane;
    p.chans = chans;
    p.h = h;
    p.w = w;
    p.oh = oh;
    p.ow = ow;
    p.nb = (w + 63) / 64;
    p.nseg = (ow + kMfSeg - 1) / kMfSeg;
    p.method = method;
    p.lds_pitch = mfma_lds_pitch(p.nb);
    p.cpr = p.lds_pitch / 16;
    p.cpr_rstep = 256 / p.cpr;
    p.cpr_dstep = 256 % p.cpr;
    p.cpr_magic = 65536 / p.cpr + 1;
    p.only_li = -1;
    return p;
}

int plain_tile_rows(int h) { return std::min(h, kMfChunkH) + kMfRows - 1; }

size_t mfma_lds_layout(MfmaParams& p, int tile_rows, size_t epi_bytes) {
    const size_t lds_main = (std::max<size_t>((size_t)tile_rows * p.lds_pitch, (size_t)kMfRows * epi_bytes) + 15) & ~(size_t)15;
    p.tc_off = (int)lds_main;
    p.st_off = (int)((lds_main + sizeof(MfTemplConst) * 32 + kMfItemBytes + 15) & ~(size_t)15);
    return (size_t)p.st_off;
}

int mfma_row_mux(MfmaParams& p, int R, int nt) {
    p.rm_R = R;
    p.rm_nt = nt;
    while ((1 << p.rm_log2nt) < nt) ++p.rm_log2nt;
    p.rm_steps = p.h + 2 * R - 1;
    p.nyb = (p.oh + 8 * R - 1) / (8 * R);
    p.ntg = 1;
    return rm_tile_rows(p.h, R);
}

int tail_split_for(const mtm_ctx* c, CallRoute& R, const SizeClass& sc) {
    if (!c->tail_screen || !c->screen_l1 || !sc.tail_ok || sc.r2 != 2 || sc.masked || sc.kernel != MTM_KERNEL_MFMA) return 0;
    if (!R.cand_on || !R.hits_only || R.ext || R.sparse || R.cand_min || c->chans != 1 || c->dtype != MTM_U8) return 0;
    if (c->method != MTM_TM_CCOEFF_NORMED && c->method != MTM_TM_CCORR_NORMED) return 0;
    if (sc.h + 1 > kMfChunkR2 || sc.w > 64) return 0;
    const double thr_lo = (double)R.cand_thr - 1e-6 * std::max(1.0, std::fabs((double)R.cand_thr));
    if (!(thr_lo >= 0.0)) return 0;
    if (c->tail_split_force > 0) return std::max(6, std::min(c->tail_split_force, sc.h - 2));
    if (R.tail_h != sc.h || R.tail_w != sc.w || R.tail_thr != R.cand_thr) {
        R.tail_s = tail_split_rule(sc.h, sc.w, thr_lo);
        R.tail_h = sc.h;
        R.tail_w = sc.w;
        R.tail_thr = R.cand_thr;
    }
    return R.tail_s;
}

static int ensure_tail_consts(mtm_ctx* c, const SizeClass& sc, int split) {
    if (split <= 0 || sc.members.empty()) return MTM_OK;
    const bool mine = !c->classes.empty() && &sc >= c->classes.data() && &sc < c->classes.data() + c->classes.size();
    const size_t k = mine ? (size_t)(&sc - c->classes.data()) : 0;
    if (mine && k < c->tail_valid.size() && c->tail_valid[k] == split) return MTM_OK;
    MTMC(launch_tail_consts(c, sc, split, c->stream));
    if (mine && k < c->tail_valid.size()) c->tail_valid[k] = split;
    return MTM_OK;
}

template <class P>
void wire_candidates(P& p, const mtm_ctx* c, const CallRoute& R, unsigned long long cap) {
    p.cand_on = R.cand_on ? 1 : 0;
    p.hits_only = (p.cand_on && R.hits_only) ? 1 : 0;
    p.cand_min = R.cand_min ? 1 : 0;
    p.cand_thr = R.cand_thr;
    p.cand_cap = cap;
    p.cand_counter = c->cands.as<unsigned long long>();
    p.cand_hits = reinterpret_cast<mtm_hit*>(c->cands.as<uint8_t>() + 16);
}

void wire_mfma_candidates(MfmaParams& p, const mtm_ctx* c, const CallRoute& R, unsigned long long cap) {
    wire_candidates(p, c, R, cap);
    p.cand_thr_lo = (double)R.cand_thr - 1e-6 * std::max(1.0, std::fabs((double)R.cand_thr));
    p.screen_hi = std::min(p.cand_thr_lo, 0.999999) - 1e-6;
    p.sq_floor = 0.99 / std::sqrt((double)p.w * (double)p.h);
    p.screen_l1 = c->screen_l1;
    if (R.cand_pin && p.cand_on && c->pinned) {
        p.cand_pin = reinterpret_cast<mtm_hit*>(static_cast<uint8_t*>(c->pinned) + 16);
        p.cand_pin_n = (unsigned long long)R.cand_pin_n;
    }
}

size_t mfma_ext_or_staging(MfmaParams& p, const mtm_ctx* c, bool ext, size_t lds) {
    if (ext) {
        p.ext_off = (int)lds;
        lds += (size_t)kMfRows * 32 * sizeof(unsigned long long);
        p.ext_best = c->counters.as<unsigned long long>();
        p.cand_on = 1;
        p.hits_only = 1;
    } else if (p.cand_on) {
        lds = (lds + 15) & ~(size_t)15;
        p.cs_off = (int)lds;
        lds += (size_t)kMfRows * kMfCandStageBytes;
    }
    return lds;
}

Bf16Params bf16_geometry(const mtm_ctx* c, const SizeClass& sc, int chans, int mb, long long group_bytes, int method) {
    const ImageDev d = image_dev(c);
    const int n = (int)sc.members.size();
    Bf16Params p{};
    p.img = d.f32;
    p.pitch = d.f32_pitch;
    p.plane = d.f32_plane;
    p.chans = chans;
    p.rows = c->rows;
    p.cols = c->cols;
    p.h = sc.h;
    p.w = sc.w;
    p.oh = c->rows - sc.h + 1;
    p.ow = c->cols - sc.w + 1;
    p.nkb = bf16_nkb(sc.w);
    p.chunk_h = p.nkb <= 2 ? 64 : 32;
    p.lds_cols = kBfSeg + 32 * p.nkb;
    p.n_list = n;
    p.nseg = (p.ow + kBfSeg - 1) / kBfSeg;
    p.nyb = (p.oh + kBfRows - 1) / kBfRows;
    p.ntg = (n + 16 * mb - 1) / (16 * mb);
    p.method = method;
    p.group_bytes = group_bytes;
    p.piece_bytes = group_bytes * mfma_groups_alloc(n);
    p.only_li = -1;
    p.n_work = p.nseg * p.nyb * p.ntg;
    return p;
}

DotParams dot_params(const mtm_ctx* c, const DotVariant& v, int chans, int h, int w, int n_list) {
    const ImageDev d = image_dev(c);
    DotParams p{};
    p.img = d.u8;
    p.pitch = d.u8_pitch;
    p.plane = d.u8_plane;
    p.chans = chans;
    p.h = h;
    p.w = w;
    p.oh = c->rows - h + 1;
    p.ow = c->cols - w + 1;
    const int w4 = (w + 3) & ~3;
    p.ncy = (h + kDotChunk - 1) / kDotChunk;
// ... 498 lines not shown
        }
        const size_t lds = mfma_lds_layout(p, tile_rows, kMfEpiBytesPerWave) + (rmr ? 0 : (size_t)kMfRows * kMfStatBytesPerWave);
        const uint8_t* ap = c->apacks.as<uint8_t>() + sl.apack_off + (rmr ? (long long)sc.slab_R * p.nb * 1024 : 0);
        if (merged && slab_s != ncc_s) HIPC(hipEventRecord(ev.first, slab_s));
        hipLaunchKernelGGL(mfma_raw_fn(rmr, false), work_grid(p.n_work), dim3(256), lds, slab_s, p, td,
                           c->tlist.as<int>() + sc.tlist_off, ap, st, maps);
        if (merged && slab_s != ncc_s) {
            HIPC(hipEventRecord(ev.second, slab_s));
            *ev_own = true;
        }
    }
    for (int i = 0; i < (merged ? 1 : n_side) && n_side > 1; ++i) {
        HIPC(hipEventRecord(c->slab_done[(size_t)i], c->slab_streams[(size_t)i]));
        HIPC(hipStreamWaitEvent(ncc_s, c->slab_done[(size_t)i], 0));
    }
    SlabParams q{};
    q.raw = c->slab_raw.as<int>();
    q.raw_slab = (long long)n_all * raw_map;
    q.raw_map = raw_map;
    q.n_slabs = S;
    q.oh = oh;
    q.ow = ow;
    q.pitch = map_pitch;
    q.n_list = n_all;
    q.method = c->method;
    q.w = w;
    q.h = h;
    q.chans = c->chans;
    wire_candidates(q, c, R, cand_list_cap(c));
    if (R.ext) {
        q.ext_on = 1;
        q.ext_best = c->counters.as<unsigned long long>();
        q.cand_on = 0;
        q.hits_only = 1;
    }
    hipLaunchKernelGGL(slab_combine_kernel, dim3((ow + 255) / 256, oh, n_all), dim3(256), 0, c->stream, q, td,
                       c->tlist.as<int>() + sc.tlist_off, st, maps, only_li);
    c->timing.kernel_used = MTM_KERNEL_MFMA;
    return MTM_OK;
}

static int launch_mfma(mtm_ctx* c, CallRoute& R, const SizeClass& sc, const StatPlanes& st, int only_li, int yb0, int yb1) {
    const int h = sc.h, w = sc.w, oh = c->rows - h + 1, ow = c->cols - w + 1;
    const int n_all = (int)sc.members.size();
    const bool rm = sc.rm_R > 0;
    const bool r2 = sc.r2 > 0;
    const int mb = r2 ? sc.r2 : (n_all > 16 || rm) ? 2 : 1;
    const int tgsz = r2 ? 16 : 16 * mb;
    MfmaParams p = mfma_geometry(c->slot[c->cur].u8b.as<uint8_t>(), image_dev(c), c->chans, h, w, oh, ow, c->method);
    p.nyb = r2 ? (oh + mb * kMfRows - 1) / (mb * kMfRows) : (oh + kMfRows - 1) / kMfRows;
    p.ntg = (n_all + tgsz - 1) / tgsz;
    p.group_bytes = sc.group_bytes;
    wire_mfma_candidates(p, c, R, (unsigned long long)c->hit_cap);
    if (p.cand_pin)
        p.clk_out = reinterpret_cast<float*>(static_cast<uint8_t*>(c->pinned) + 8);
    else if (p.cand_on && c->cands.p)
        p.clk_out = reinterpret_cast<float*>(c->cands.as<uint8_t>() + 8);
    if (R.sparse) {
        p.seg_flags = c->seg_flags.as<uint8_t>();
        p.flag_tstride = R.flag_tstride;
        p.flag_rstride = R.flag_rstride;
        const bool normed_m = c->method == MTM_TM_SQDIFF_NORMED || c->method == MTM_TM_CCORR_NORMED || c->method == MTM_TM_CCOEFF_NORMED;
        p.seg_skip = (c->seg_skip && !sc.masked && normed_m) ? 1 : 0;
        R.seg_skip_used = R.seg_skip_used || p.seg_skip != 0;
    }
    int tg0 = 0;
    if (only_li >= 0 && !rm) {
        tg0 = only_li / tgsz;
        p.ntg = 1;
    }
    int tile_rows = r2 ? std::min(h + mb - 1, kMfChunkR2) + (kMfRows - 1) * mb : plain_tile_rows(h);
    if (rm) {
        tile_rows = mfma_row_mux(p, sc.rm_R, sc.rm_nt);
        p.rm_cstride = class_rm_pack_bytes(sc);
        p.rm_rsq = c->stats_rsq.as<double>();
    }
    if (yb1 >= 0) {
        p.yb0 = yb0;
        p.nyb = std::min(yb1, p.nyb) - yb0;
    }
    p.n_work = p.nseg * p.nyb * p.ntg;
    p.tail_split = (r2 && st.blkq != nullptr && only_li < 0 && !p.seg_skip) ? tail_split_for(c, R, sc) : 0;
    MTMC(ensure_tail_consts(c, sc, p.tail_split));
    if (!c->classes.empty() && &sc >= c->classes.data() && &sc < c->classes.data() + c->classes.size() &&
        (size_t)(&sc - c->classes.data()) < c->tail_last.size())
        c->tail_last[(size_t)(&sc - c->classes.data())] = p.tail_split;
    const size_t stat_bytes = rm ? 0 : r2 ? (size_t)kMfRows * ((mb + 1) / 2) * 1024 + (p.tail_split ? mf_tail_lds_bytes() : 0)
                                          : (size_t)kMfRows * mf_stat_bytes_per_wave(c->chans == 3 ? 3 : 1);
    const bool ext = R.ext;
    const size_t lds = mfma_ext_or_staging(p, c, ext, mfma_lds_layout(p, tile_rows, kMfEpiBytesPerWave) + stat_bytes);
    p.kp_nseg = sc.kp_nseg;
    p.kp_blocks = sc.kp_nseg ? kp_blocks(h, sc.kp_nseg) : 0;
    const uint8_t* ap = c->apacks.as<uint8_t>() + sc.apack_off +
                        (rm ? (sc.kp_nseg ? 0LL : (long long)sc.rm_R * p.nb * 1024)
                            : (long long)tg0 * (r2 ? 1 : mb) * sc.group_bytes);
    p.n_list = n_all - tg0 * tgsz;
    if (only_li >= 0) p.only_li = only_li - tg0 * tgsz;
    const int* tl_k = c->tlist.as<int>() + sc.tlist_off + tg0 * tgsz;
    MfmaSel sel;
    sel.mb = mb;
    sel.masked = sc.masked;
    sel.rm = rm;
    sel.ch = (c->chans == 3 && !sc.masked) ? 3 : 1;
    sel.method = (c->chans == 1 || sel.ch == 3) ? c->method : -1;
    sel.ext = ext;
    sel.exact_div = c->exact_div != 0 && !(ext && sc.masked);
    sel.r2 = r2;
    sel.kp = sc.kp_nseg > 0;
    const MfmaFn fn = mfma_kernel(sel);
    if (!fn) {
        set_error("internal: no ncc_mfma_kernel instantiation for this class");
        return MTM_E_STATE;
    }
    hipLaunchKernelGGL(fn, work_grid(p.n_work), dim3(256), lds, c->stream, p, c->td.as<TemplDev>(), tl_k, ap, st,
                       c->maps.as<float>());
    c->timing.kernel_used = MTM_KERNEL_MFMA;
    return MTM_OK;
}

static int launch_mfma16(mtm_ctx* c, CallRoute& R, const SizeClass& sc, const StatPlanes& st, int only_li, int yb0, int yb1) {
    const int h = sc.h, w = sc.w, oh = c->rows - h + 1, ow = c->cols - w + 1;
    const int n_all = (int)sc.members.size(), n_pad = sc.n_pad;
    MfmaParams p = mfma_geometry(c->slot[c->cur].u8b.as<uint8_t>(), image_dev(c), 2, h, w, oh, ow, c->method);
    p.nyb = (oh + kMfRows - 1) / kMfRows;
    p.ntg = n_pad / 16;
    p.group_bytes = sc.group_bytes;
    int tg0 = 0;
    if (only_li >= 0) {
        tg0 = only_li / 16;
        p.ntg = 1;
    }
    if (yb1 >= 0) {
        p.yb0 = yb0;
        p.nyb = std::min(yb1, p.nyb) - yb0;
    }
    p.n_work = p.nseg * p.nyb * p.ntg;
    p.kp_nseg = sc.kp_nseg;
    p.kp_blocks = sc.kp_nseg ? kp_blocks(h, sc.kp_nseg) : 0;
    p.n_list = n_all - tg0 * 16;
    if (only_li >= 0) p.only_li = only_li - tg0 * 16;
    p.u16_tsum = c->tsum.as<double>() + sc.tsum_off + tg0 * 16;
    p.u16_npad = n_pad;
    p.u16_area = (double)h * (double)w;
    wire_mfma_candidates(p, c, R, cand_list_cap(c));
    const bool ext = R.ext;
    const size_t lds = mfma_ext_or_staging(p, c, ext, mfma_lds_layout(p, plain_tile_rows(h), kMfU16EpiBytesPerWave));
    const uint8_t* ap = c->apacks.as<uint8_t>() + sc.apack_off + (long long)tg0 * 2 * sc.group_bytes;
    const int* tl_k = c->tlist.as<int>() + sc.tlist_off + tg0 * 16;
    MfmaSel sel16;
    sel16.method = kMfU16;
    sel16.kp = sc.kp_nseg > 0;
    sel16.ext = ext;
    sel16.exact_div = c->exact_div != 0;
    hipLaunchKernelGGL(mfma_kernel(sel16), work_grid(p.n_work), dim3(256), lds, c->stream, p, c->td.as<TemplDev>(), tl_k, ap,
                       st, c->maps.as<float>());
    c->timing.kernel_used = MTM_KERNEL_MFMA16;
    return MTM_OK;
}

static int launch_bf16(mtm_ctx* c, CallRoute& R, const SizeClass& sc, const StatPlanes& st, int only_li, int yb0, int yb1) {
    const int h = sc.h;
    const int n_all = (int)sc.members.size();
    const int mb = n_all > 16 ? 2 : 1;
    Bf16Params p = bf16_geometry(c, sc, c->chans, mb, sc.group_bytes, c->method);
    if (yb1 >= 0) {
        p.yb0 = yb0;
        p.nyb = std::min(yb1, p.nyb) - yb0;
    }
    int tg0 = 0;
// ... 619 lines not shown
```

multitemplatematching-python_amd/csrc/mtm_mfma.hip.h:

```cpp
#pragma once
#include "mtm_device_util.hip.h"
#include "mtm_mfma_params.h"

namespace mtm {

__device__ __forceinline__ int mf_epi_rot(int j) { return 4 * ((j >> 1) & 3); }
__device__ __forceinline__ int mf_opaque_sgpr(int v) {
    asm volatile("" : "+s"(v));
    return v;
}
template <int METHOD>
__device__ __forceinline__ float finish_vals(int method_rt, double corr, const double (&t)[kMaxChans], double sum2,
                                             double sq, const MfTemplConst& T, int chans) {
    const int method = METHOD >= 0 ? METHOD : method_rt;
    if (T.all_ones) return 1.0f;
    if (method == MTM_TM_CCORR) return (float)corr;
    const int num_type = (method == MTM_TM_CCORR_NORMED) ? 0
                       : (method == MTM_TM_CCOEFF || method == MTM_TM_CCOEFF_NORMED) ? 1 : 2;
    const bool normed = (method == MTM_TM_SQDIFF_NORMED) || (method == MTM_TM_CCORR_NORMED) ||
                        (method == MTM_TM_CCOEFF_NORMED);
    double num = corr;
    if (num_type == 1) {
#pragma unroll
        for (int c = 0; c < kMaxChans; ++c)
// ... 105 lines not shown
}

template <int METHOD, bool EXACT_DIV, bool DEFER = false>
__device__ __forceinline__ float finish_lean_masked(int a32, double p1, double c2, double rsqrt_c2,
                                                    const MfTemplConst& T, bool* redo = nullptr) {
    const double c1 = (double)a32 + (p1 + T.mfma_k);
    if (METHOD == MTM_TM_CCORR) return (float)c1;
    if (METHOD == MTM_TM_SQDIFF) return (float)(-2.0 * c1 + c2 + T.tms);
    const double num = (METHOD == MTM_TM_SQDIFF_NORMED) ? (-2.0 * c1 + c2 + T.tms) : c1;
    if constexpr (EXACT_DIV && DEFER) {
        const double q0 = num * (rsqrt_c2 * T.rsqrt_tms);
        const bool finite = ((uint32_t)__double2hiint(q0) & 0x7ff00000u) != 0x7ff00000u;
        *redo = quotient_needs_division<true>(q0) || !finite;
        return (float)q0;
    }
    return EXACT_DIV ? (float)(num / sqrt(T.tms * c2)) : (float)(num * (rsqrt_c2 * T.rsqrt_tms));
}

template <int MB>
__device__ __forceinline__ void mfma_step(v4i (&acc)[MB][16], const v4i qa, const v4i qb, const v4i (&a)[MB]) {
    const int W[8] = {qa.x, qa.y, qa.z, qa.w, qb.x, qb.y, qb.z, qb.w};
#pragma unroll
    for (int cq = 0; cq < 4; ++cq) {
        const v4i bv = {W[cq], W[cq + 1], W[cq + 2], W[cq + 3]};
#pragma unroll
        for (int mb = 0; mb < MB; ++mb)
            acc[mb][4 * cq] = __builtin_amdgcn_mfma_i32_16x16x64_i8(a[mb], bv, acc[mb][4 * cq], 0, 0, 0);
    }
#pragma unroll
    for (int cr = 1; cr < 4; ++cr) {
        int E[7];
#pragma unroll
        for (int m = 0; m < 7; ++m) E[m] = (int)__builtin_amdgcn_alignbyte((uint32_t)W[m + 1], (uint32_t)W[m], cr);
#pragma unroll
        for (int cq = 0; cq < 4; ++cq) {
            const v4i bv = {E[cq], E[cq + 1], E[cq + 2], E[cq + 3]};
#pragma unroll
            for (int mb = 0; mb < MB; ++mb)
                acc[mb][4 * cq + cr] =
                    __builtin_amdgcn_mfma_i32_16x16x64_i8(a[mb], bv, acc[mb][4 * cq + cr], 0, 0, 0);
        }
    }
}

#ifndef MTM_MFMA_NO_ASM
#include "mtm_mfma_step_asm.inc"
#else
__device__ __forceinline__ void mfma_step_one_set(v4i (&acc)[2][16], const v4i qa, const v4i qb, const v4i (&a)[2]) {
    mfma_step<2>(acc, qa, qb, a);
}
#endif
#ifndef MTM_STEP_VARIANT
#define MTM_STEP_VARIANT 2
#endif
__device__ __forceinline__ void mfma_step2(v4i (&acc)[2][16], const v4i qa, const v4i qb, const v4i (&a)[2]) {
#if defined(MTM_MFMA_NO_ASM) || MTM_STEP_VARIANT == 0
    mfma_step<2>(acc, qa, qb, a);
#elif MTM_STEP_VARIANT == 2
    mfma_step2_fused_b(acc, qa, qb, a);
#else
    mfma_step2_fused(acc, qa, qb, a);
#endif
}
__device__ __forceinline__ void mfma_step2_rm(v4i (&acc)[2][16], const v4i qa, const v4i qb, const v4i (&a)[2], const int mode) {
#if defined(MTM_MFMA_NO_ASM) || MTM_STEP_VARIANT == 0
    if (mode == 0) {
        mfma_step<2>(acc, qa, qb, a);
    } else {
        v4i (&acc1)[1][16] = reinterpret_cast<v4i (&)[1][16]>(acc[mode - 1]);
        const v4i a1[1] = {a[mode - 1]};
        mfma_step<1>(acc1, qa, qb, a1);
    }
#else
    mfma_step2_edges(acc, qa, qb, a, mode);
#endif
}
template <int METHOD_, int MB>
__device__ __forceinline__ void mfma_kstep(v4i (&acc)[MB][16], const v4i qa, const v4i qb, const v4i (&a)[MB]) {
    if constexpr (METHOD_ == 7 && MB == 2) mfma_step_one_set(acc, qa, qb, a);
    else if constexpr (MB == 2) mfma_step2(acc, qa, qb, a);
    else mfma_step<MB>(acc, qa, qb, a);
}

template <int MB, int METHOD, bool EXACT_DIV, bool MASKED = false, bool RM = false, int CH = 1, bool EXT = false,
          bool R2 = false, bool KP = false>
__global__ __launch_bounds__(256, 2) void ncc_mfma_kernel(MfmaParams p, const TemplDev* __restrict__ td,
                                                          const int* __restrict__ tlist,
                                                          const uint8_t* __restrict__ apack,
                                                          StatPlanes st, float* __restrict__ maps) {
    constexpr bool C1 = METHOD >= 0;
    static_assert(CH == 1 || !MASKED, "multi-channel: unmasked paths only");
    static_assert(!EXT || (METHOD >= 0 && METHOD != kMfRaw), "fused extremum: compile-time-method paths");
    static_assert(METHOD != kMfU16 || (MB == 2 && !MASKED && !RM && CH == 1 && !R2), "uint16 finishing pass");
    static_assert(!KP || (!R2 && METHOD >= 0 && (METHOD != kMfRaw || !RM)), "packed K");
    static_assert(!R2 || (MB == 2 && METHOD >= 2 && METHOD <= 5 && !MASKED && !RM && CH == 1), "two-row variant");
    static_assert(MB <= 2, "at most two MFMA groups per wave");
    extern __shared__ __attribute__((aligned(16))) uint8_t smem[];

    int* s_item = reinterpret_cast<int*>(smem + p.tc_off + 32 * (int)sizeof(MfTemplConst));
    const bool clk_probe = p.clk_out != nullptr && blockIdx.x == (gridDim.x >> 1) && threadIdx.x == 0;
    if (clk_probe) {
        unsigned long long* clk0 = reinterpret_cast<unsigned long long*>(s_item + 4);
        clk0[0] = __builtin_readcyclecounter();
        clk0[1] = __builtin_amdgcn_s_memrealtime();
    }
    const int per_xcd = (p.n_work + 7) >> 3;
    do {
    const int wid = (blockIdx.x & 7) * per_xcd + (blockIdx.x >> 3);
    if (wid >= p.n_work) break;
    if (!EXT && METHOD != kMfRaw && p.hits_only) {
        if (threadIdx.x == 0)
            s_item[2] = __hip_atomic_load(p.cand_counter, __ATOMIC_RELAXED, __HIP_MEMORY_SCOPE_AGENT) > p.cand_cap ? 1 : 0;
        __syncthreads();
        if (s_item[2]) break;
    }
    const int tg = wid % p.ntg;
    const int rest = wid / p.ntg;
    const int seg = rest % p.nseg;
    int yb = rest / p.nseg;
    long long slab_img = 0, slab_ap = 0, slab_raw = 0;
    if constexpr (RM && METHOD == kMfRaw && !KP) {
        if (p.n_slab > 1) {
            const int k = yb / p.nyb;
            yb -= k * p.nyb;
            const int cb = k % p.slab_ncb, rbk = k / p.slab_ncb;
            const int rb = rbk % p.slab_nrb, ch = rbk / p.slab_nrb;
            slab_img = (long long)ch * p.plane + (long long)rb * p.slab_rh * p.pitch + (long long)cb * p.slab_cw;
            slab_ap = (long long)k * p.slab_ap_step;
            slab_raw = (long long)k * p.slab_raw_step;
        }
    }
    const int x0 = seg * kMfSeg, y0 = (yb + p.yb0) * (RM ? 8 * p.rm_R : (R2 ? MB * kMfRows : kMfRows));
    int tid_i = threadIdx.x;
    asm volatile("" : "+v"(tid_i));
    const int wave = __builtin_amdgcn_readfirstlane(tid_i >> 6), lane = tid_i & 63;
    const int j = lane & 15, q = lane >> 4;
    const int wave_rows = RM ? 2 * p.rm_R : (R2 ? MB : 1);
    constexpr int kTG = R2 ? 16 : 16 * MB;

    v4i acc[MB][16];
#pragma unroll
    for (int mb = 0; mb < MB; ++mb)
#pragma unroll
        for (int c = 0; c < 16; ++c) acc[mb][c] = v4i{0, 0, 0, 0};
    v4i u16_hh[METHOD == kMfU16 ? 16 : 1];

    MfTemplConst* tcl = reinterpret_cast<MfTemplConst*>(smem + p.tc_off);
    constexpr int kTGc = METHOD == kMfU16 ? 16 : kTG;
    if (METHOD != kMfRaw && tid_i < (RM ? p.rm_nt : kTGc)) {
        const int li = tg * kTGc + tid_i;
        if (li < p.n_list) {
            const TemplDev& T = td[tlist[li]];
            MfTemplConst k;
#pragma unroll
            for (int cc = 0; cc < kMaxChans; ++cc) k.mean[cc] = T.mean[cc];
            k.templ_norm = T.templ_norm;
            k.templ_sum2 = T.templ_sum2;
            k.mfma_k = T.mfma_k;
            if constexpr (METHOD == kMfU16) {
                const double kh = 128.0 * p.u16_tsum[li] - 16384.0 * p.u16_area;
                const double kl = 128.0 * p.u16_tsum[p.u16_npad + li] - 16384.0 * p.u16_area;
                k.mfma_k = 257.0 * (256.0 * kh + kl);
            }
            k.rtempl_norm = T.templ_norm > 0.0 ? 1.0 / T.templ_norm : 0.0;
#pragma unroll
            for (int cc = 0; cc < kMaxChans; ++cc) k.m128[cc] = 128.0 - T.mean[cc];
            k.tms = T.templ2_mask2_sum;
            k.rsqrt_tms = 1.0 / sqrt(T.templ2_mask2_sum);
            k.map_off = T.map_off;
            k.map_pitch = T.map_pitch;
            k.all_ones = T.all_ones;
            {
                int ninf_hi = (int)0xfff00000;
                asm volatile("" : "+v"(ninf_hi));
                k.ext_thr_lo = __hiloint2double(ninf_hi, 0);
            }
            k.ext_hi = 0u;
            k.flag_base = tlist[li] * p.flag_tstride;
            if (EXT) {
                const unsigned long long bk = __hip_atomic_load(&p.ext_best[2 * tlist[li] + p.cand_min], __ATOMIC_RELAXED,
                                                                __HIP_MEMORY_SCOPE_AGENT);
                if (bk) {
                    const uint32_t hiw = (uint32_t)(bk >> 32);
                    const double sc = (double)mf_order_float(p.cand_min ? ~hiw : hiw);
                    const double ql = p.cand_min ? -sc : sc;
                    k.ext_hi = hiw;
                    k.ext_thr_lo = ql - 1e-6 * fmax(1.0, fabs(ql));
                }
            }
            tcl[tid_i] = k;
        } else if (!RM) {
            MfTemplConst k;
#pragma unroll
            for (int cc = 0; cc < kMaxChans; ++cc) k.mean[cc] = 0.0, k.m128[cc] = 0.0;
            k.templ_norm = 1.0;
            k.templ_sum2 = 0.0;
            k.mfma_k = -1e300;
            k.rtempl_norm = 0.0;
            k.tms = 1.0;
            k.rsqrt_tms = 0.0;
            k.map_off = 0;
            k.map_pitch = 0;
            k.all_ones = 0;
            k.ext_thr_lo = 1e300;
            k.ext_hi = 0xFFFFFFFFu;
            k.flag_base = 0;
            tcl[tid_i] = k;
        }
    }

    if constexpr (R2 && !EXT && (METHOD == MTM_TM_CCORR_NORMED || METHOD == MTM_TM_CCOEFF_NORMED)) {
        if (mf_opaque_sgpr(p.tail_split) > 0 && tid_i < 16) {
            MfTailConst* ttl = reinterpret_cast<MfTailConst*>(smem + p.st_off + kMfRows * ((MB + 1) / 2) * 1024 + kMfTailRecBytes);
            const int li = tg * 16 + tid_i;
            MfTailConst k;
            if (li < p.n_list) {
                const TemplDev& T = td[tlist[li]];
#pragma unroll
                for (int r = 0; r < 2; ++r) k.k[r] = T.tail_k[r], k.d[r] = T.tail_d[r], k.g[r] = T.tail_g[r];
            } else {
#pragma unroll
                for (int r = 0; r < 2; ++r) k.k[r] = -1e300, k.d[r] = 0.0, k.g[r] = 0.0;
            }
            ttl[tid_i] = k;
        }
    }

    constexpr bool kNeedSum2 = MASKED || METHOD == MTM_TM_SQDIFF || METHOD == MTM_TM_SQDIFF_NORMED;
    constexpr bool kNormed = !MASKED && (METHOD == MTM_TM_SQDIFF_NORMED || METHOD == MTM_TM_CCORR_NORMED ||
                                         METHOD == MTM_TM_CCOEFF_NORMED);
    constexpr bool kMaskedNormed = MASKED && (METHOD == MTM_TM_SQDIFF_NORMED || METHOD == MTM_TM_CCORR_NORMED);
    if constexpr (R2 && kNormed) {
        typedef const __attribute__((address_space(1))) void* gptr_t;
        typedef __attribute__((address_space(3))) void* lptr_t;
        uint8_t* sbase = smem + p.st_off + wave * (((MB + 1) / 2) * 1024);
        const int bj = min((x0 >> 4) + ((lane & 31) >> 1), st.blk_pitch - 1);
#pragma unroll
        for (int r0 = 0; r0 < MB; r0 += 2) {
            const int yr = min(y0 + MB * wave + min(r0 + (lane >> 5), MB - 1), p.oh - 1);
            const double* src = st.blk + ((size_t)yr * st.blk_pitch + bj) * 4 + 2 * (lane & 1);
            __builtin_amdgcn_global_load_lds((gptr_t)src, (lptr_t)(sbase + (r0 / 2) * 1024), 16, 0, 0);
        }
        if (!EXT && mf_opaque_sgpr(p.tail_split) > 0) {
#pragma unroll
            for (int r0 = 0; r0 < MB; r0 += 2) {
                const int yr = min(y0 + MB * wave + min(r0 + (lane >> 5), MB - 1), p.oh - 1);
                const double* src = st.blkq + ((size_t)yr * st.blk_pitch + bj) * 4 + 2 * (lane & 1);
                __builtin_amdgcn_global_load_lds((gptr_t)src, (lptr_t)(sbase + kMfRows * ((MB + 1) / 2) * 1024 + (r0 / 2) * 1024),
                                                 16, 0, 0);
            }
        }
    } else if constexpr (C1 && METHOD != kMfRaw && METHOD != kMfU16 && !RM && !R2) {
        typedef const __attribute__((address_space(1))) void* gptr_t;
        typedef __attribute__((address_space(3))) void* lptr_t;
        const int yc = min(y0 + wave, p.oh - 1), xc = min(x0 + 4 * lane, st.pitch - 4);
        const size_t sidx = (size_t)yc * st.pitch + xc;
        uint8_t* sbase = smem + p.st_off + wave * mf_stat_bytes_per_wave(CH);
#pragma unroll
        for (int hh = 0; hh < 2; ++hh) {
#pragma unroll
            for (int cc = 0; cc < CH; ++cc)
                __builtin_amdgcn_global_load_lds((gptr_t)(st.t[cc] + sidx + 2 * hh), (lptr_t)(sbase + (2 * cc + hh) * 1024), 16, 0, 0);
            if (kNeedSum2)
                __builtin_amdgcn_global_load_lds((gptr_t)(st.sum2 + sidx + 2 * hh), (lptr_t)(sbase + (2 * CH + hh) * 1024), 16, 0, 0);
            if (kNormed)
                __builtin_amdgcn_global_load_lds((gptr_t)(st.sq + sidx + 2 * hh), (lptr_t)(sbase + (2 * CH + 2 + hh) * 1024), 16, 0, 0);
        }
    }

    const uint8_t* apack_g = apack + slab_ap + (long long)tg * (R2 ? 1 : MB) * p.group_bytes + (size_t)lane * 16;
    bool tail_out = false;

    for (int c = 0; c < p.chans; ++c) {
        const uint8_t* plane = p.img + slab_img + c * p.plane;
        const int cpk = (METHOD == kMfU16 || (RM && METHOD == kMfRaw && p.sq_fused)) ? 0 : c;
        if constexpr (RM && METHOD == kMfRaw && !KP) {
            if (p.sq_fused && c == 1) {
#pragma unroll
                for (int mb = 0; mb < MB; ++mb)
#pragma unroll
                    for (int k = 0; k < 16; ++k) acc[mb][k] = acc[mb][k] * 256;
            }
        }
        if constexpr (METHOD == kMfU16) {
            if (c == 1) {
#pragma unroll
                for (int k = 0; k < 16; ++k) {
                    u16_hh[k] = acc[0][k];
                    acc[0][k] = acc[1][k];
                    acc[1][k] = v4i{0, 0, 0, 0};
                }
            }
        }
        const int krows = RM ? p.rm_steps : (R2 ? p.h + MB - 1 : p.h);
        constexpr int kChunk = R2 ? kMfChunkR2 : kMfChunkH;
        v4i r2_prev = v4i{0, 0, 0, 0};
        for (int cy0 = 0; cy0 < krows; cy0 += kChunk) {
            const int ch = min(kChunk, krows - cy0);
            __syncthreads();
            {
                typedef const __attribute__((address_space(1))) void* gptr_t;
                typedef __attribute__((address_space(3))) void* lptr_t;
                const int nchunk = (ch + (kMfRows - 1) * wave_rows) * p.cpr;
                int ci = tid_i;
                int r = (ci * p.cpr_magic) >> 16, d = ci - r * p.cpr;
                const uint8_t* grow = plane + (size_t)(y0 + cy0) * p.pitch + x0;
                uint8_t* lbase_w = smem + wave * 1024;
                for (; ci - lane < nchunk; ci += 256) {
                    if (ci < nchunk)
                        __builtin_amdgcn_global_load_lds((gptr_t)(grow + (size_t)r * p.pitch + 16 * d), (lptr_t)lbase_w,
                                                         16, 0, 0);
                    lbase_w += 4096;
                    r += p.cpr_rstep;
                    d += p.cpr_dstep;
                    if (d >= p.cpr) {
                        d -= p.cpr;
                        ++r;
                    }
                }
                asm volatile("s_waitcnt vmcnt(0)" ::: "memory");
            }
            __syncthreads();
            if constexpr (R2) {
                const uint8_t* aptr = apack_g + (size_t)cy0 * 1024;
                const uint8_t* lbase = smem + wave * wave_rows * p.lds_pitch + (j + q) * 16;
                int loff = 0;
                v4i qx, qy, qx2, qy2, aA, aB, aC = r2_prev;
                if (mf_opaque_sgpr(p.hits_only)) __builtin_amdgcn_s_setprio(3);
#define MTM_R2_LOAD(QA, QB, A)                                              \
                QA = *reinterpret_cast<const v4i*>(lbase + loff);           \
                QB = *reinterpret_cast<const v4i*>(lbase + loff + 16);      \
                A = *reinterpret_cast<const v4i*>(aptr);
#define MTM_R2_STEP(QA, QB, ACUR, APREV, QA2, QB2, ANEXT)                   \
                {                                                           \
                    aptr += 1024;                                           \
                    loff += p.lds_pitch;                                    \
                    MTM_R2_LOAD(QA2, QB2, ANEXT)                            \
                    __builtin_amdgcn_sched_barrier(0);                      \
                    const v4i ar_[2] = {ACUR, APREV};                       \
                    mfma_step2(acc, QA, QB, ar_);                           \
                    __builtin_amdgcn_sched_barrier(0);                      \
                }
#define MTM_R2_STEP_LAST(QA, QB, ACUR, APREV)                               \
                {                                                           \
                    aptr += 1024;                                           \
                    loff += p.lds_pitch;                                    \
                    __builtin_amdgcn_sched_barrier(0);                      \
                    const v4i ar_[2] = {ACUR, APREV};                       \
                    mfma_step2(acc, QA, QB, ar_);                           \
                    __builtin_amdgcn_sched_barrier(0);                      \
                }
#define MTM_R2_FIVE()                                                        \
                MTM_R2_STEP(qx, qy, aA, aC, qx2, qy2, aB)                   \
                MTM_R2_STEP(qx2, qy2, aB, aA, qx, qy, aC)                   \
                MTM_R2_STEP(qx, qy, aC, aB, qx2, qy2, aA)                   \
                MTM_R2_STEP(qx2, qy2, aA, aC, qx, qy, aB)                   \
                MTM_R2_STEP(qx, qy, aB, aA, qx2, qy2, aC)
                MTM_R2_LOAD(qx, qy, aA)
                int ks = 0;
                const int split = (!EXT && kNormed) ? mf_opaque_sgpr(p.tail_split) : 0;
                if (split > 0) {
                    for (; ks + 6 < split; ks += 6) {
                        MTM_R2_FIVE()
                        MTM_R2_STEP(qx2, qy2, aC, aB, qx, qy, aA)
                    }
#pragma nounroll
                    for (; ks + 1 < split; ++ks) {
                        MTM_R2_STEP(qx, qy, aA, aC, qx2, qy2, aB)
                        aC = aA;
                        aA = aB;
                        qx = qx2;
                        qy = qy2;
                    }
                    MTM_R2_STEP_LAST(qx, qy, aA, aC)
                    aC = aA;
                    ks = split;
                    asm volatile("s_nop 15\n\ts_nop 15" ::: "memory");
                    bool pass = false;
                    const uint8_t* sbw = smem + p.st_off + wave * 1024 + j * 32;
                    const uint8_t* sbq = sbw + kMfRows * 1024;
                    const MfTailConst* ttl = reinterpret_cast<const MfTailConst*>(smem + p.st_off + 2 * kMfRows * 1024);
#pragma unroll
                    for (int mb = 0; mb < MB; ++mb) {
                        int amax[4] = {INT_MIN, INT_MIN, INT_MIN, INT_MIN};
#pragma unroll
                        for (int c = 0; c < 16; ++c) {
                            const v4i a = acc[mb][c];
                            amax[0] = max(amax[0], a.x);
                            amax[1] = max(amax[1], a.y);
                            amax[2] = max(amax[2], a.z);
                            amax[3] = max(amax[3], a.w);
                        }
                        const double2 s1 = *reinterpret_cast<const double2*>(sbw + mb * 512);
                        const double sq_eff = fmax(*reinterpret_cast<const double*>(sbw + mb * 512 + 16), p.sq_floor);
                        const double2 s1q = *reinterpret_cast<const double2*>(sbq + mb * 512);
                        const double vq = *reinterpret_cast<const double*>(sbq + mb * 512 + 16);
#pragma unroll
                        for (int e = 0; e < 4; ++e) {
                            const MfTemplConst& T = tcl[4 * q + e];
                            const MfTailConst& U = ttl[4 * q + e];
                            const double m = METHOD == MTM_TM_CCOEFF_NORMED ? T.m128[0] : 128.0;
                            const double dq = U.d[mb];
                            const double bound = (((double)amax[e] + U.k[mb]) + fmax(m * s1.x, m * s1.y)) +
                                                 fmax(dq * s1q.x, dq * s1q.y) + vq * U.g[mb];
                            pass = pass || T.all_ones != 0 || bound > p.screen_hi * T.templ_norm * sq_eff;
                        }
                    }
                    tail_out = __builtin_amdgcn_ballot_w64(pass) == 0ull;
                    if (!tail_out) { MTM_R2_LOAD(qx, qy, aA) }
                }
                if (!tail_out) {
                    for (; ks + 6 <= ch; ks += 6) {
                        MTM_R2_FIVE()
                        MTM_R2_STEP(qx2, qy2, aC, aB, qx, qy, aA)
                    }
                    r2_prev = aC;
                    if (ks < ch) { MTM_R2_STEP(qx, qy, aA, aC, qx2, qy2, aB) r2_prev = aA; }
                    if (ks + 1 < ch) { MTM_R2_STEP(qx2, qy2, aB, aA, qx, qy, aC) r2_prev = aB; }
                    if (ks + 2 < ch) { MTM_R2_STEP(qx, qy, aC, aB, qx2, qy2, aA) r2_prev = aC; }
                    if (ks + 3 < ch) { MTM_R2_STEP(qx2, qy2, aA, aC, qx, qy, aB) r2_prev = aA; }
                    if (ks + 4 < ch) { MTM_R2_STEP(qx, qy, aB, aA, qx2, qy2, aC) r2_prev = aB; }
                }
#undef MTM_R2_LOAD
#undef MTM_R2_STEP
#undef MTM_R2_STEP_LAST
#undef MTM_R2_FIVE
                asm volatile("s_nop 15\n\ts_nop 15" ::: "memory");
                __builtin_amdgcn_s_setprio(0);
            } else if constexpr (KP) {
            const int nseg = p.kp_nseg;
            const uint8_t* aptr = apack_g + (RM ? (size_t)cpk * p.rm_cstride : (size_t)cpk * p.kp_blocks * 1024) +
                                  (size_t)((cy0 * nseg) >> 2) * 1024;
            const uint8_t* lbase = smem + wave * wave_rows * p.lds_pitch + j * 16;
            const int nsteps = (ch * nseg + 3) >> 2;
            const int drow = 4 / nseg, dseg = 4 - drow * nseg;
            const int adv = drow * p.lds_pitch + dseg * 16, wrapfix = p.lds_pitch - nseg * 16;
            int seg = q % nseg;
            int loff = (q / nseg) * p.lds_pitch + seg * 16;
            v4i qa0, qb0, qa1, qb1, a0[MB], a1[MB];
#define MTM_KP_ADVANCE()                                            \
            {                                                       \
// ... 980 lines not shown
                            if constexpr (!EXT) if (p.seg_flags != nullptr) {
                                if (__builtin_amdgcn_ballot_w64(above) != 0ull)
                                    p.seg_flags[(size_t)T.flag_base + (size_t)yrow * p.flag_rstride + (x0 >> 8)] = 1;
                            }
                        }
                    }
                }
                __builtin_amdgcn_fence(__ATOMIC_SEQ_CST, "wavefront");
                __builtin_amdgcn_wave_barrier();
            }
        }
        if (EXT && lane < kTG) {
            const unsigned long long key = ext_slot[lane];
            const int li = tg * kTG + lane;
            if (key && li < p.n_list) atomicMax(&p.ext_best[2 * tlist[li] + p.cand_min], key);
        }
    } else {
        __syncthreads();
#pragma unroll 1
        for (int stage = 0; stage < 2 * MB; ++stage) {
            const int mb = stage >> 1, round = stage & 1;
            if ((q >> 1) == round) {
                if (mb == 0) put(acc[0]);
                else put(acc[MB - 1]);
            }
            __builtin_amdgcn_fence(__ATOMIC_SEQ_CST, "wavefront");
            __builtin_amdgcn_wave_barrier();
            {
                const bool lane_on = y < p.oh && xq < p.ow;
#pragma unroll 1
                for (int s8 = 0; s8 < 8; ++s8) {
                    const int lt = mb * 16 + 8 * round + s8;
                    const int li = tg * MB * 16 + lt;
                    if (li >= p.n_list) break;
                    if (p.only_li >= 0 && li != p.only_li) continue;
                    const MfTemplConst T = tcl[lt];
                    const v4i a4 = *reinterpret_cast<const v4i*>(&epi[s8 * kMfEpiPitch + rd_off]);
                    const int a32[4] = {a4.x, a4.y, a4.z, a4.w};
                    float out[4];
#pragma unroll
                    for (int i = 0; i < 4; ++i) {
                        const int x = min(xq + i, p.ow - 1);
                        const size_t sidx = (size_t)min(y, p.oh - 1) * st.pitch + x;
                        double tv[kMaxChans] = {0.0, 0.0, 0.0, 0.0};
                        double s1 = 0.0;
#pragma unroll
                        for (int cc = 0; cc < kMaxChans; ++cc)
                            if (cc < p.chans) {
                                tv[cc] = st.t[cc][sidx];
                                s1 += tv[cc];
                            }
                        const double corr = ((double)a32[i] + 128.0 * s1) + T.mfma_k;
                        out[i] = finish_vals<-1>(p.method, corr, tv, st.sum2[sidx], st.sq[sidx], T, p.chans);
                    }
                    if (p.cand_on) emit_at(out, li, y, lane_on ? 15u : 0u);
                    if (lane_on) store4(maps + T.map_off + (size_t)y * T.map_pitch + xq, out);
                }
            }
            __builtin_amdgcn_fence(__ATOMIC_SEQ_CST, "wavefront");
            __builtin_amdgcn_wave_barrier();
        }
    }
    if (cs_on) {
        __builtin_amdgcn_fence(__ATOMIC_SEQ_CST, "wavefront");
        __builtin_amdgcn_wave_barrier();
        const int n_st = __builtin_amdgcn_readfirstlane(cs_cnt[0]);
        if (n_st > 0) {
            unsigned long long base = 0ull;
            if (lane == 0) base = atomicAdd(p.cand_counter, (unsigned long long)n_st);
            const uint32_t blo = __builtin_amdgcn_readfirstlane((uint32_t)base);
            const uint32_t bhi = __builtin_amdgcn_readfirstlane((uint32_t)(base >> 32));
            base = ((unsigned long long)bhi << 32) | blo;
                for (int r = lane; r < n_st; r += 64)
                    mf_put_cand(p, base + (unsigned long long)r, cs_rec[r]);
        }
    }
    }
    } while (false);
    if (p.clk_out != nullptr && blockIdx.x == (gridDim.x >> 1) && threadIdx.x == 0) {
        const unsigned long long* clk0 = reinterpret_cast<const unsigned long long*>(s_item + 4);
        const unsigned long long dt = __builtin_readcyclecounter() - clk0[0], dr = __builtin_amdgcn_s_memrealtime() - clk0[1];
        if (dr > 0) *p.clk_out = (float)((double)dt * 100.0 / (double)dr);
    }
}

}
```

multitemplatematching-python_amd/csrc/mtm_mfma_params.h:

```cpp
#pragma once
#include <hip/hip_runtime.h>
#include <cstdint>

#include "mtm_kernels.h"
#include "../../include/mtm_hip.h"

namespace mtm {

typedef int v4i __attribute__((ext_vector_type(4)));

constexpr int kMfSeg = 256;
constexpr int kMfRows = 4;
constexpr int kMfChunkH = 64;
constexpr int kMfChunkR2 = 72;
constexpr int kMfEpiPitch = 260;
constexpr int kMfEpiBytesPerWave = 8 * kMfEpiPitch * 4;
constexpr int kMfU16EpiBytesPerWave = 12 * kMfEpiPitch * 4;
constexpr int kMfStatPlaneBytes = 2 * 1024;
constexpr int kMfStatBytesPerWave = 3 * kMfStatPlaneBytes;
__host__ __device__ constexpr int mf_stat_bytes_per_wave(int ch) { return (ch + 2) * kMfStatPlaneBytes; }
constexpr int kMfItemBytes = 32;
constexpr int kMfCandStage = 128;
constexpr int kMfCandStageBytes = 16 + kMfCandStage * 24;
constexpr int kMfRaw = 6;
constexpr int kMfU16 = 7;

struct MfmaParams {
    const uint8_t* img;
    int pitch;
    long long plane;
    int chans;
    int h, w;
    int oh, ow;
    int nb;
    int n_list;
    int nseg, nyb, ntg;
    int yb0;
    int n_work;
    int method;
    int lds_pitch;
    int cpr, cpr_rstep, cpr_dstep;
    int cpr_magic, cpr_pad_;
    long long group_bytes;
    int only_li;
    int tc_off;
    int st_off;
    int pad0_[4];
    mtm_hit* cand_hits;
    unsigned long long* cand_counter;
    unsigned long long cand_cap;
    float cand_thr;
    int cand_min;
    int cand_on;
    int rm_R, rm_nt, rm_log2nt, rm_steps;
    long long rm_cstride;
    const double* rm_rsq;
    int n_slab, slab_ncb, slab_nrb, slab_cw, slab_rh;
    long long slab_ap_step, slab_raw_step;
    int* raw_out;
    long long raw_map;
    int raw_pitch;
    double cand_thr_lo;
    double screen_hi;
    double sq_floor;
    int screen_l1, screen_pad_;
    int hits_only;
    int ext_off;
    unsigned long long* ext_best;
    int dbg_unused_;
    int kp_nseg;
    int kp_blocks;
    const double* u16_tsum;
    int u16_npad, u16_pad_;
    double u16_area;
    int cs_off;
    int sq_fused;
    int pad_rm_edges_;
    uint8_t* seg_flags;
    int flag_tstride, flag_rstride;
    int seg_skip;
    double sq_k;
    float* clk_out;
    mtm_hit* cand_pin;
    unsigned long long cand_pin_n;
    int tail_split;
    int tail_pad_;
};

__device__ __forceinline__ void mf_put_cand(const MfmaParams& p, unsigned long long slot, const mtm_hit& h) {
    if (slot < p.cand_cap) p.cand_hits[slot] = h;
    if (slot < p.cand_pin_n) p.cand_pin[slot] = h;
}

struct MfTemplConst {
    double mean[kMaxChans];
    double templ_norm, templ_sum2, mfma_k;
    double rtempl_norm;
    double m128[kMaxChans];
    double tms, rsqrt_tms;
    long long map_off;
    int map_pitch, all_ones;
    double ext_thr_lo;
    unsigned ext_hi;
    int flag_base;
};
struct MfTailConst {
    double k[2], d[2], g[2];
};
constexpr int kMfTailRecBytes = kMfRows * 1024;
constexpr int mf_tail_lds_bytes() { return kMfTailRecBytes + 16 * (int)sizeof(MfTailConst); }

using MfmaFn = void (*)(MfmaParams, const TemplDev*, const int*, const uint8_t*, StatPlanes, float*);

struct MfmaSel {
    int mb = 2;
    int method = 0;
    bool exact_div = false;
    bool masked = false;
    bool rm = false;
    int ch = 1;
    bool ext = false;
    bool r2 = false;
    bool kp = false;
};
MfmaFn mfma_kernel(const MfmaSel& s);
MfmaFn mfma_kernel_plain(const MfmaSel& s);
MfmaFn mfma_kernel_rm(const MfmaSel& s);
MfmaFn mfma_kernel_ext(const MfmaSel& s);
MfmaFn mfma_kernel_kp(const MfmaSel& s);
MfmaFn mfma_kernel_rows(const MfmaSel& s);

}
```

multitemplatematching-python_amd/csrc/mtm_placement.hip:

```cpp
#include <functional>
#include "mtm_ctx.h"

using namespace mtm;
using namespace mtmi;
#include "mtm_templates.hip.h"

namespace {

size_t dot_pack_bytes(int h, int w, int chans) {
    const int w4 = (w + 3) & ~3;
    const int ncy = (h + kDotChunk - 1) / kDotChunk, ncx = (w4 + kDotChunk - 1) / kDotChunk;
    return (size_t)chans * ncy * ncx * kDotChunkBytes;
}

void pack_template_dot4(const HostTempl& t, uint8_t* out) {
    const int h = t.rows, w = t.cols;
    const int w4 = (w + 3) & ~3;
    const int ncy = (h + kDotChunk - 1) / kDotChunk, ncx = (w4 + kDotChunk - 1) / kDotChunk;
    std::memset(out, 0, dot_pack_bytes(h, w, t.chans));
    for (int c = 0; c < t.chans; ++c)
        for (int cy = 0; cy < ncy; ++cy)
            for (int cx = 0; cx < ncx; ++cx) {
                uint8_t* chunk = out + ((size_t)(c * ncy + cy) * ncx + cx) * kDotChunkBytes;
                const int ch = std::min(kDotChunk, h - cy * kDotChunk);
// ... 331 lines not shown
        p.chans = 1;
        p.h = sc.h + sc.r2 - 1;
        p.group_bytes = sc.group_bytes;
        p.n_chunks = p.group_bytes * ((p.n + 15) / 16) / 16;
    } else {
        p.mode = 0;
        p.chans = c->chans;
        p.group_bytes = sc.group_bytes;
        p.kblocks = sc.kp_nseg ? kp_blocks(sc.h, sc.kp_nseg) : 0;
        p.n_chunks = p.group_bytes * mfma_groups_alloc(p.n) / 16;
    }
    launch(sc.apack_off);
    HIPC(hipGetLastError());
    return MTM_OK;
}

struct Bump {
    size_t size = 0;
    long long take(size_t n) {
        size += n;
        return (long long)(size - n);
    }
};

struct Placement {
    std::vector<SizeClass> classes;
    std::vector<char> dev_pack;
    std::vector<size_t> a_bytes;
    std::vector<int> host_px;
    std::vector<TemplDev> td, td_u, td_v;
    std::vector<int> tlist, list2d;
    int list2d_off = 0;
    std::vector<UnitSrc> units;
    Bump maps, w, p, a, ts;
    bool any_host_pack = false, any_mbf = false;
};

void choose_tiling(const mtm_ctx* c, SizeClass& sc) {
    const int n_cls = (int)sc.members.size(), nseg = (sc.w + 15) / 16;
    sc.rm_nt = sc.rm_R = sc.slab_nt = sc.slab_R = sc.r2 = sc.kp_nseg = 0;
    sc.slabs.clear();
    if (sc.kernel == MTM_KERNEL_MFMA16) sc.kp_nseg = nseg % 4 != 0 ? nseg : 0;
    if (sc.kernel != MTM_KERNEL_MFMA) return;
    if (sc.w > kMfmaMaxW || (long long)c->chans * sc.w * sc.h > 131071) {
        sc.slabs = slab_layout(c, sc);
        if (n_cls <= 16) {
            int hs = 0, ws = 0;
            for (const auto& sl : sc.slabs) {
                hs = std::max(hs, sl.r1 - sl.r0);
                ws = std::max(ws, sl.c1 - sl.c0);
            }
            sc.slab_nt = rm_group_templates(n_cls, hs, ws);
            sc.slab_R = 16 / sc.slab_nt;
        }
        return;
    }
    const bool one_pack = c->chans == 1 || (c->chans == 3 && !sc.masked);
    if (c->row_mux && n_cls <= 16 && c->fuse_stats && one_pack && (double)c->chans * sc.w * sc.h * 65025.0 < 4294967296.0) {
        sc.rm_nt = rm_group_templates(n_cls, sc.h, sc.w);
        sc.rm_R = 16 / sc.rm_nt;
    }
    const bool normed = c->method == MTM_TM_SQDIFF_NORMED || c->method == MTM_TM_CCORR_NORMED ||
                        c->method == MTM_TM_CCOEFF_NORMED;
    if (nseg % 4 != 0 && normed && one_pack && (!sc.masked || c->method != MTM_TM_CCOEFF_NORMED))
        sc.kp_nseg = nseg;
    else if (c->mfma_r2 && sc.rm_R == 0 && n_cls > 16 && sc.w <= 64 && c->chans == 1 && !sc.masked &&
             c->method >= MTM_TM_CCORR && c->fuse_stats)
        sc.r2 = 2;
    if (sc.r2 == 2 && sc.h + 1 <= mtm::kMfChunkR2 && sc.h >= 8) {
        sc.tail_ok = true;
        sc.tail_split = c->tail_split_force > 0 ? std::max(6, std::min(c->tail_split_force, sc.h - 2))
                                                : tail_split_rule(sc.h, sc.w, kTailDefaultThr - 1e-6);
    }
}

int queue_tail_consts(mtm_ctx* c, const SizeClass& sc, int split, hipStream_t stream) {
    hipLaunchKernelGGL(tail_consts_kernel, dim3((unsigned)sc.members.size()), dim3(64), 0, stream,
                       c->apacks.as<uint8_t>() + sc.apack_off, sc.group_bytes, sc.h, sc.w, split,
                       c->tlist.as<int>() + sc.tlist_off, c->td.as<TemplDev>());
    HIPC(hipGetLastError());
    return MTM_OK;
}

size_t place_apacks(const mtm_ctx* c, SizeClass& sc, Bump& a, Bump& ts) {
    const int n_cls = (int)sc.members.size(), groups = mfma_groups_alloc(n_cls);
    size_t bytes = 0;
    switch (sc.kernel) {
        case MTM_KERNEL_MFMA:
            sc.mask_rm_off = -1;
            if (sc.masked && c->row_mux && c->fuse_stats) {
                sc.mask_rm_off = a.take((size_t)rm_pack_bytes(sc.h, sc.w, 16));
                const HostTempl& m0 = c->templs[sc.members[0]];
                sc.mask_ones = m0.on_device ? m0.mask_ones : 0.0;
                if (!m0.on_device)
                    for (double m : m0.mask) sc.mask_ones += m > 0.0 ? 1.0 : 0.0;
            }
            if (!sc.slabs.empty()) {
                sc.apack_off = (long long)a.size;
                for (auto& sl : sc.slabs) {
                    const int hs = sl.r1 - sl.r0, ws = sl.c1 - sl.c0;
                    sl.apack_off = a.take(sc.slab_R > 0 ? (size_t)rm_pack_bytes(hs, ws, sc.slab_R)
                                                        : (size_t)mfma_group_bytes(hs, ws, 1) * groups);
                }
                return 0;
            }
            if (sc.rm_R > 0) {
                sc.group_bytes = sc.kp_nseg ? class_rm_pack_bytes(sc) / 2
                                            : -(long long)sc.rm_R * ((sc.w + 63) / 64) * 1024;
                bytes = (size_t)class_rm_pack_bytes(sc) * (sc.masked ? 1 : c->chans);
            } else if (sc.r2) {
                sc.group_bytes = mfma_group_bytes(sc.h + sc.r2 - 1, sc.w, 1);
                bytes = (size_t)sc.group_bytes * ((n_cls + 15) / 16);
            } else {
                sc.group_bytes = sc.kp_nseg ? (long long)c->chans * kp_blocks(sc.h, sc.kp_nseg) * 1024
                                            : mfma_group_bytes(sc.h, sc.w, c->chans);
                bytes = (size_t)sc.group_bytes * groups;
            }
            break;
        case MTM_KERNEL_MFMA_F32:
            sc.group_bytes = bf16_group_bytes(sc.h, sc.w, c->chans);
            bytes = (size_t)(2 * sc.group_bytes * groups);
            break;
        case MTM_KERNEL_MFMA16:
            sc.group_bytes = sc.kp_nseg ? (long long)kp_blocks(sc.h, sc.kp_nseg) * 1024 : mfma_group_bytes(sc.h, sc.w, 1);
            bytes = (size_t)sc.group_bytes * (2 * sc.n_pad / 16);
            sc.tsum_off = ts.take(2 * (size_t)sc.n_pad);
            break;
        default:
            if (!sc.mask_bf16) return 0;
            sc.mbf_group_bytes = bf16_group_bytes(sc.h, sc.w, 1);
            bytes = (size_t)(2 * sc.mbf_group_bytes * groups);
            sc.mbf_off_u = a.take(bytes);
            sc.mbf_off_v = a.take(bytes);
            return bytes;
    }
    sc.apack_off = a.take(bytes);
    return bytes;
}

int plan_placement(const mtm_ctx* c, Placement& P) {
    const int n = (int)c->templs.size();
    P.classes = c->classes;
    for (SizeClass& sc : P.classes) {
        sc.kernel = resolved_kernel(c, sc);
        sc.n_pad = (int)round_up(sc.members.size(), 16);
        choose_tiling(c, sc);
        sc.masked_int = sc.masked && sc.kernel == MTM_KERNEL_MFMA;
        sc.mask_bf16 = sc.kernel == MTM_KERNEL_AUTO && masked_bf16_class_ok(c, sc);
        sc.mbf_off_u = sc.mbf_off_v = sc.tsum_off = -1;
    }
    P.td.assign((size_t)n, TemplDev{});
    for (int i = 0; i < n; ++i) {
        const HostTempl& t = c->templs[i];
        const int kern = P.classes[(size_t)t.cls].kernel;
        if (t.chans != c->chans) {
            set_error("template " + std::to_string(i) + " has a different channel count than the image");
            return MTM_E_INVALID;
        }
        if (t.rows > c->rows || t.cols > c->cols) {
            set_error("template " + std::to_string(i) + " is larger than the image");
            return MTM_E_INVALID;
        }
        TemplDev& d = P.td[i];
        for (int k = 0; k < kMaxChans; ++k) d.mean[k] = t.st.mean[k];
        d.templ_norm = t.st.templ_norm;
        d.templ_sum2 = t.st.templ_sum2;
// ... 81 lines not shown
    std::vector<double> wts, tsums;
    std::vector<uint8_t> packs, apacks;
};
void pack_on_host(const mtm_ctx* c, Placement& P, HostArenas& H) {
    H.wts.resize(P.w.size);
    H.packs.resize(P.p.size);
    H.apacks.resize(P.any_host_pack ? P.a.size : 0);
    H.tsums.resize(P.ts.size);
    uint8_t* a = H.apacks.data();
    for (size_t i = 0; i < P.td.size(); ++i) {
        const HostTempl& t = c->templs[i];
        const TemplDev& d = P.td[i];
        if (d.k1_off >= 0 && t.masked) {
            for (size_t k = 0; k < t.px.size(); ++k) {
                const double m2 = t.mask[k] * t.mask[k];
                H.wts[d.k1_off + k] = t.px[k] * m2;
                H.wts[d.k2_off + k] = m2;
            }
        } else if (d.k1_off >= 0) {
            std::copy(t.px.begin(), t.px.end(), H.wts.begin() + d.k1_off);
        }
        if (d.pack_off >= 0) pack_template_dot4(t, H.packs.data() + d.pack_off);
    }
    for (size_t k = 0; k < P.classes.size(); ++k) {
        const SizeClass& sc = P.classes[k];
        if (sc.mask_pack_off >= 0) {
            HostTempl mk = c->templs[sc.members[0]];
            for (size_t q = 0; q < mk.px.size(); ++q) mk.px[q] = mk.mask[q] > 0.0 ? 255.0 : 0.0;
            pack_template_dot4(mk, H.packs.data() + sc.mask_pack_off);
        }
        if (sc.mask_bf16) {
            pack_class_bf16(c, sc, a + sc.mbf_off_u, sc.mbf_group_bytes, P.a_bytes[k], P.td_u, 1);
            pack_class_bf16(c, sc, a + sc.mbf_off_v, sc.mbf_group_bytes, P.a_bytes[k], P.td_v, 2);
        }
        if (P.dev_pack[k]) continue;
        if (sc.kernel == MTM_KERNEL_MFMA && sc.mask_rm_off >= 0) pack_mask_rm(c, sc, a + sc.mask_rm_off);
        if (sc.kernel == MTM_KERNEL_MFMA && sc.rm_R > 0)
            pack_class_rm(c, sc, a + sc.apack_off, P.a_bytes[k]);
        else if (sc.kernel == MTM_KERNEL_MFMA)
            pack_class_mfma(c, sc, a + sc.apack_off, P.a_bytes[k]);
        if (sc.kernel == MTM_KERNEL_MFMA16) pack_class_mfma16(c, sc, a + sc.apack_off, P.a_bytes[k], H.tsums.data() + sc.tsum_off);
        if (sc.kernel == MTM_KERNEL_MFMA_F32) pack_class_bf16(c, sc, a + sc.apack_off, sc.group_bytes, P.a_bytes[k], P.td, 0);
    }
}

int upload_placement(mtm_ctx* c, Placement& P, HostArenas& H) {
    struct DrainGuard {
        hipStream_t s;
        bool armed = true;
        ~DrainGuard() {
            if (armed) (void)hipStreamSynchronize(s);
        }
    } drain{c->stream};
    const size_t n = P.td.size(), a_off = P.a.size, w_off = P.w.size, p_off = P.p.size, ts_off = P.ts.size;
    const bool new_units = P.units.size() > c->usrc_units;
    if (new_units) {
        MTMC(c->usrc_dev.ensure(sizeof(UnitSrc) * P.units.size()));
        HIPC(hipMemcpyAsync(c->usrc_dev.p, P.units.data(), sizeof(UnitSrc) * P.units.size(), hipMemcpyHostToDevice, c->stream));
    }
    MTMC(c->td.ensure(sizeof(TemplDev) * n));
    MTMC(c->tlist.ensure(sizeof(int) * std::max<size_t>(1, P.tlist.size())));
    MTMC(c->weights.ensure(sizeof(double) * std::max<size_t>(1, w_off)));
    MTMC(c->packs.ensure(std::max<size_t>(4, p_off)));
    MTMC(c->apacks.ensure(std::max<size_t>(16, a_off) + 16384));
    if (a_off && P.any_host_pack) HIPC(hipMemcpyAsync(c->apacks.p, H.apacks.data(), a_off, hipMemcpyHostToDevice, c->stream));
    HIPC(hipMemcpyAsync(c->td.p, P.td.data(), sizeof(TemplDev) * n, hipMemcpyHostToDevice, c->stream));
    if (!P.tlist.empty())
        HIPC(hipMemcpyAsync(c->tlist.p, P.tlist.data(), sizeof(int) * P.tlist.size(), hipMemcpyHostToDevice, c->stream));
    if (w_off) HIPC(hipMemcpyAsync(c->weights.p, H.wts.data(), sizeof(double) * w_off, hipMemcpyHostToDevice, c->stream));
    if (p_off) HIPC(hipMemcpyAsync(c->packs.p, H.packs.data(), p_off, hipMemcpyHostToDevice, c->stream));
    if (P.any_mbf) {
        MTMC(c->td_u.ensure(sizeof(TemplDev) * n));
        MTMC(c->td_v.ensure(sizeof(TemplDev) * n));
        HIPC(hipMemcpyAsync(c->td_u.p, P.td_u.data(), sizeof(TemplDev) * n, hipMemcpyHostToDevice, c->stream));
        HIPC(hipMemcpyAsync(c->td_v.p, P.td_v.data(), sizeof(TemplDev) * n, hipMemcpyHostToDevice, c->stream));
    }
    MTMC(c->tsum.ensure(sizeof(double) * std::max<size_t>(2, ts_off)));
    if (ts_off) HIPC(hipMemcpyAsync(c->tsum.p, H.tsums.data(), sizeof(double) * ts_off, hipMemcpyHostToDevice, c->stream));
    for (size_t k = 0; k < P.classes.size(); ++k)
        if (P.dev_pack[k]) MTMC(pack_class_on_device(c, P.classes[k]));
    for (const SizeClass& sc : P.classes)
        if (sc.tail_split > 0 && sc.kernel == MTM_KERNEL_MFMA && !sc.members.empty())
            MTMC(queue_tail_consts(c, sc, sc.tail_split, c->stream));
    const bool local_sources = P.any_host_pack || P.any_mbf || w_off || p_off || ts_off || new_units;
    if (local_sources) HIPC(hipStreamSynchronize(c->stream));
    c->place_pending = !local_sources;
    drain.armed = false;
    if (new_units) c->usrc_host.swap(P.units);
    c->classes.swap(P.classes);
    c->tail_valid.assign(c->classes.size(), 0);
    c->tail_last.assign(c->classes.size(), 0);
    for (size_t k = 0; k < c->classes.size(); ++k) {
        const SizeClass& sc = c->classes[k];
        if (sc.tail_split > 0 && sc.kernel == MTM_KERNEL_MFMA && !sc.members.empty()) c->tail_valid[k] = sc.tail_split;
    }
    c->td_host.swap(P.td);
    c->tlist_host.swap(P.tlist);
    c->list2d.swap(P.list2d);
    c->list2d_off = P.list2d_off;
    c->maps_floats = P.maps.size;
    c->placed = true;
    return MTM_OK;
}

}

namespace mtmi {

int launch_tail_consts(mtm_ctx* c, const SizeClass& sc, int split, hipStream_t stream) { return queue_tail_consts(c, sc, split, stream); }

int place_templates(mtm_ctx* c) {
    if (!c->have_image || !c->have_templ) {
        set_error("set the image and the templates first");
        return MTM_E_STATE;
    }
    if (c->placed) return MTM_OK;
    if (c->place_pending) {
        HIPC(hipStreamSynchronize(c->stream));
        c->place_pending = false;
    }
    Placement P;
    MTMC(plan_placement(c, P));
    for (int i : P.host_px) MTMC(ensure_host_pixels(c, i));
    HostArenas H;
    pack_on_host(c, P, H);
    return upload_placement(c, P, H);
}

int parse_templ_blob(const std::vector<uint8_t>& b, std::vector<BlobTempl>& out, const char* who, bool u16_ok) {
    size_t off = 0;
    auto rd = [&](void* dst, size_t n) {
        if (off + n > b.size()) return false;
        std::memcpy(dst, b.data() + off, n);
        off += n;
        return true;
    };
    int n_templ = 0, method = 0, n_var = 0;
    if (!rd(&n_templ, sizeof(int)) || !rd(&method, sizeof(int)) || !rd(&n_var, sizeof(int))) {
        set_error(std::string(who) + ": no templates set");
        return MTM_E_STATE;
    }
    if (n_var != 0) {
        set_error(std::string(who) + ": takes the templates of mtm_set_templates (not an augmented set)");
        return MTM_E_INVALID;
    }
    out.clear();
    for (int i = 0; i < n_templ; ++i) {
        int hdr[5];
        if (!rd(hdr, sizeof(hdr))) return MTM_E_STATE;
        const bool u16 = u16_ok && hdr[3] == MTM_U16 && hdr[2] == 1;
        if ((hdr[3] != MTM_U8 && !u16) || hdr[4] != 0) {
            set_error(std::string(who) + ": template " + std::to_string(i) +
                      (u16_ok ? " is not an unmasked uint8 or single-channel uint16 template"
                              : " is not an unmasked uint8 template"));
            return MTM_E_INVALID;
        }
        const size_t bytes = (size_t)hdr[0] * hdr[1] * hdr[2] * (u16 ? 2 : 1);
        if (off + bytes > b.size()) return MTM_E_STATE;
        out.push_back(BlobTempl{hdr[0], hdr[1], hdr[2], hdr[3], b.data() + off});
        off += bytes;
    }
    return MTM_OK;
}

int prepare_window_templates(mtm_ctx* c, const std::vector<BlobTempl>& tl) {
    if (c->win_gen != c->templ_gen && !c->win_blob.empty() && c->win_blob == c->templ_blob) {
        if (c->pyr_gen == c->win_gen) c->pyr_gen = c->templ_gen;
        if (c->box_gen == c->win_gen) c->box_gen = c->templ_gen;
        c->win_gen = c->templ_gen;
    }
    if (c->win_gen == c->templ_gen) return MTM_OK;
    c->win_gen = 0;
    c->win_blob.clear();
    const size_t n = tl.size();
    std::vector<uint8_t> planar;
    std::vector<long long> toff(n, 0);
    for (size_t i = 0; i < n; ++i) {
        const BlobTempl& t = tl[i];
        const size_t plane = (size_t)t.rows * t.cols;
        toff[i] = (long long)planar.size();
        if (t.dtype == MTM_U16) {
            planar.resize(planar.size() + 2 * plane);
            uint8_t* dst = planar.data() + toff[i];
            for (size_t p = 0; p < plane; ++p) {
                uint16_t v;
                std::memcpy(&v, t.px + 2 * p, sizeof(v));
                dst[p] = (uint8_t)(v >> 8);
                dst[plane + p] = (uint8_t)(v & 255u);
            }
        } else {
            planar.resize(planar.size() + plane * t.chans);
            uint8_t* dst = planar.data() + toff[i];
// ... 440 lines not shown
```

multitemplatematching-python_amd/csrc/mtm_templates.hip.h:

```cpp
#pragma once
#include <hip/hip_runtime.h>
#include <cstdint>

#include "mtm_kernels.h"
#include "mtm_templates_params.h"

namespace mtm {


__device__ __forceinline__ unsigned unit_px(const uint8_t* __restrict__ arena, const UnitSrc& u, int c, int y, int x) {
    const int sy = u.ay * y + u.by * x + u.cy, sx = u.ax * y + u.bx * x + u.cx;
    return arena[u.off + ((long long)c * u.sh + sy) * u.sw + sx];
}
__device__ __forceinline__ unsigned unit_mask(const uint8_t* __restrict__ arena, const UnitSrc& u, int c, int y, int x) {
    const int sy = u.ay * y + u.by * x + u.cy, sx = u.ax * y + u.bx * x + u.cx;
    return arena[u.moff + ((long long)c * u.sh + sy) * u.sw + sx] > 0 ? 1u : 0u;
}

__global__ void resize_area_kernel(const uint8_t* __restrict__ src, int sh, int sw, uint8_t* __restrict__ dst, int dh,
                                   int dw, int planes) {
    const int j = blockIdx.x * blockDim.x + threadIdx.x, i = blockIdx.y, p = blockIdx.z;
    if (j >= dw || i >= dh || p >= planes) return;
    const uint8_t* s = src + (size_t)p * sh * sw;
    const long long ylo = (long long)i * sh, yhi = (long long)(i + 1) * sh;
    const long long xlo = (long long)j * sw, xhi = (long long)(j + 1) * sw;
    long long num = 0;
    for (long long y = ylo / dh; y < sh && y * dh < yhi; ++y) {
        const long long wy = min(yhi, (y + 1) * dh) - max(ylo, y * dh);
        if (wy <= 0) continue;
        long long row = 0;
        for (long long x = xlo / dw; x < sw && x * dw < xhi; ++x) {
            const long long wx = min(xhi, (x + 1) * dw) - max(xlo, x * dw);
            if (wx > 0) row += wx * (long long)s[y * sw + x];
        }
        num += wy * row;
    }
    const long long den = (long long)sh * sw;
    const long long v = (2 * num + den) / (2 * den);
    dst[(size_t)p * dh * dw + (size_t)i * dw + j] = (uint8_t)(v < 0 ? 0 : (v > 255 ? 255 : v));
}

__global__ void downscale_int_kernel(const uint8_t* __restrict__ src, int sh, int sw, uint8_t* __restrict__ dst, int f,
                                     int planes) {
    const int dh = sh / f, dw = sw / f;
    const int j = blockIdx.x * blockDim.x + threadIdx.x, i = blockIdx.y, p = blockIdx.z;
    if (j >= dw || i >= dh || p >= planes) return;
    const uint8_t* s = src + (size_t)p * sh * sw;
    unsigned sum = 0;
    for (int dy = 0; dy < f; ++dy)
        for (int dx = 0; dx < f; ++dx) sum += s[(size_t)(i * f + dy) * sw + (size_t)j * f + dx];
    const float scale = 1.0f / (float)(f * f);
    const unsigned r = (f == 2) ? ((sum + 2u) >> 2) : (unsigned)rintf((float)sum * scale);
    dst[(size_t)p * dh * dw + (size_t)i * dw + j] = (uint8_t)(r > 255u ? 255u : r);
}


__global__ __launch_bounds__(256) void source_sums_kernel(const uint8_t* __restrict__ arena,
                                                          const SourceDesc* __restrict__ srcs,
                                                          unsigned long long* __restrict__ out) {
    const SourceDesc d = srcs[blockIdx.x];
    __shared__ unsigned long long red[4][kSumsPerSource];
    const long long n = (long long)d.sh * d.sw;
    unsigned long long acc[kSumsPerSource];
#pragma unroll
    for (int k = 0; k < kSumsPerSource; ++k) acc[k] = 0ull;
    for (int c = 0; c < d.chans; ++c)
        for (long long i = threadIdx.x; i < n; i += 256) {
            const unsigned long long v = arena[d.off + c * n + i];
            const unsigned long long m = d.moff >= 0 ? (arena[d.moff + c * n + i] > 0 ? 1ull : 0ull) : 0ull;
            acc[4 * c + 0] += v;
            acc[4 * c + 1] += v * v;
            acc[4 * c + 2] += v * m;
            acc[4 * c + 3] += v * v * m;
            if (c == 0) acc[4 * kMaxChans] += m;
        }
#pragma unroll
    for (int k = 0; k < kSumsPerSource; ++k) {
        unsigned long long v = acc[k];
        for (int off = 32; off > 0; off >>= 1) v += __shfl_down(v, off);
        if ((threadIdx.x & 63) == 0) red[threadIdx.x >> 6][k] = v;
    }
    __syncthreads();
    if (threadIdx.x < kSumsPerSource)
        out[(size_t)blockIdx.x * kSumsPerSource + threadIdx.x] =
            red[0][threadIdx.x] + red[1][threadIdx.x] + red[2][threadIdx.x] + red[3][threadIdx.x];
}

// ... 28 lines not shown
    r /= p.nb;
    if (p.mode == 0) {
        dy = (int)(r % p.h);
        r /= p.h;
        ch = (int)(r % p.chans);
        const int g = (int)(r / p.chans);
        li = 16 * g + i;
    } else {
        const int steps = p.h + 3 * p.R - 1;
        const int sp = (int)(r % steps);
        ch = (int)(r / steps);
        const int t = p.mode == 2 ? 0 : i % p.nt, rho = p.mode == 2 ? i : i / p.nt;
        dy = sp - p.R - rho;
        li = t;
    }
    }
    uint32_t wds[4] = {0u, 0u, 0u, 0u};
    if (li >= 0 && li < p.n && dy >= 0 && dy < p.hv) {
        const UnitSrc u = units[tl[li]];
#pragma unroll
        for (int byte = 0; byte < 16; ++byte) {
            const int dx = 64 * b + 16 * qtap + byte;
            if (dx < p.w) {
                unsigned v;
                if (p.mode == 2) v = unit_mask(arena, u, 0, dy, dx);
                else {
                    v = unit_px(arena, u, ch, dy, dx);
                    if (p.masked) v *= unit_mask(arena, u, ch, dy, dx);
                }
                wds[byte >> 2] |= ((p.mode == 2 ? v : (v ^ 0x80u)) & 255u) << (8 * (byte & 3));
            }
        }
    }
    *reinterpret_cast<uint4*>(out + k * 16) = make_uint4(wds[0], wds[1], wds[2], wds[3]);
}

__global__ void gather_unit_kernel(const uint8_t* __restrict__ arena, UnitSrc u, uint8_t* __restrict__ px,
                                   uint8_t* __restrict__ mask) {
    const int x = blockIdx.x * blockDim.x + threadIdx.x, y = blockIdx.y, c = blockIdx.z;
    if (x >= u.w || y >= u.h) return;
    const size_t o = ((size_t)c * u.h + y) * u.w + x;
    px[o] = (uint8_t)unit_px(arena, u, c, y, x);
    if (mask != nullptr) mask[o] = u.moff >= 0 ? (uint8_t)unit_mask(arena, u, c, y, x) : 0;
}

constexpr int kTailMaxRows = 128;
__global__ __launch_bounds__(64) void tail_consts_kernel(const uint8_t* __restrict__ apack, long long group_bytes, int h, int w,
                                                         int split, const int* __restrict__ tl, TemplDev* __restrict__ td) {
    __shared__ long long rs[kTailMaxRows][2];
    const int li = blockIdx.x, r = threadIdx.x;
    const uint8_t* g = apack + (size_t)(li / 16) * group_bytes;
    for (int y = r; y < h; y += 64) {
        long long s = 0, s2 = 0;
        for (int x = 0; x < w; ++x) {
            const long long v = g[((size_t)y * 64 + 16 * (x / 16) + li % 16) * 16 + x % 16] ^ 0x80;
            s += v;
            s2 += v * v;
        }
        rs[y][0] = s;
        rs[y][1] = s2;
    }
    __syncthreads();
    if (r >= 2) return;
    const int q0 = r == 0 ? split : split - 1;
    long long sall = 0, sq = 0, s2q = 0;
    for (int y = 0; y < h; ++y) {
        sall += rs[y][0];
        if (y >= q0) {
            sq += rs[y][0];
            s2q += rs[y][1];
        }
    }
    const long long nq = (long long)(h - q0) * w, np = (long long)q0 * w, n = (long long)h * w;
    const double kp = 128.0 * (double)(sall - sq) - 16384.0 * (double)np;
    const double d = (double)sq / (double)nq - 128.0;
    const double gg = sqrt((double)(nq * s2q - sq * sq) / (double)nq) * (1.0 + 0x1p-49);
    const double mag = 4294967296.0 + fabs(kp) + 2.0 * 128.0 * 255.0 * (double)n + gg * 128.0 * sqrt((double)nq);
    TemplDev& t = td[tl[li]];
    t.tail_k[r] = kp + mag * 0x1p-46;
    t.tail_d[r] = d;
    t.tail_g[r] = gg;
}

}
```

Baseline: 420,000.

## Prepack per-group template constants and stage them via LDS DMA with first tile

After: 417,600. Within noise of the previous version (-0.6%).

```diff
diff --git a/include/mtm_hip.h b/include/mtm_hip.h
--- a/include/mtm_hip.h
+++ b/include/mtm_hip.h
@@ -111,6 +111,7 @@
 int         mtm_debug_templ_stats(const void* px, int rows, int cols, int chans, int dtype, int method, double* out7);
 #define MTM_CLASS_TILING_FIELDS 12
 int         mtm_debug_class_tilings(mtm_ctx* ctx, int32_t* out, int cap_classes);
+int         mtm_debug_tc_pack(mtm_ctx* ctx, int32_t* out, int cap_classes);
 int         mtm_debug_device_nms(mtm_ctx* ctx, const mtm_hit* hits, int64_t n, int rows, int cols, int max_side,
                                  double score_threshold, int ascending, double max_overlap, int64_t n_min, int64_t n_max,
                                  mtm_hit* out, int64_t capacity, int64_t* n_champions, int64_t* n_undecided);
diff --git a/multitemplatematching-python_amd/MTM/_lib.py b/multitemplatematching-python_amd/MTM/_lib.py
--- a/multitemplatematching-python_amd/MTM/_lib.py
+++ b/multitemplatematching-python_amd/MTM/_lib.py
@@ -106,6 +106,7 @@
     "mtm_debug_quotient_check": (ctypes.c_int, [ctypes.c_void_p, ctypes.c_uint64, ctypes.c_uint64, _P(ctypes.c_uint64)]),
     "mtm_debug_tail_split": (ctypes.c_int, [ctypes.c_int, ctypes.c_int, ctypes.c_double]),
     "mtm_debug_class_tilings": (ctypes.c_int, [ctypes.c_void_p, _P(ctypes.c_int32), ctypes.c_int]),
+    "mtm_debug_tc_pack": (ctypes.c_int, [ctypes.c_void_p, _P(ctypes.c_int32), ctypes.c_int]),
     "mtm_debug_templ_stats": (ctypes.c_int, [ctypes.c_void_p, ctypes.c_int, ctypes.c_int, ctypes.c_int, ctypes.c_int,
                                              ctypes.c_int, _P(ctypes.c_double)]),
     "mtm_debug_device_nms": (ctypes.c_int, [ctypes.c_void_p, ctypes.c_void_p, ctypes.c_int64, ctypes.c_int, ctypes.c_int,
@@ -494,6 +495,13 @@
         check(min(self._lib.mtm_debug_class_tilings(self._h, buf, n), 0), "mtm_debug_class_tilings")
         return [dict(zip(CLASS_TILING_FIELDS, buf[k * nf:(k + 1) * nf])) for k in range(n)]
 
+    def tc_pack_state(self):
+        n = self._lib.mtm_debug_tc_pack(self._h, None, 0)
+        check(min(n, 0), "mtm_debug_tc_pack")
+        buf = (ctypes.c_int32 * (2 * max(n, 1)))()
+        check(min(self._lib.mtm_debug_tc_pack(self._h, buf, n), 0), "mtm_debug_tc_pack")
+        return [{"valid": int(buf[2 * k]), "used": int(buf[2 * k + 1])} for k in range(n)]
+
     def debug_quotient_check(self, n_cases=1 << 28, seed=1):
         out = (ctypes.c_uint64 * 4)()
         check(self._lib.mtm_debug_quotient_check(self._h, int(n_cases), int(seed), out), "mtm_debug_quotient_check")
diff --git a/multitemplatematching-python_amd/csrc/mtm_context.hip b/multitemplatematching-python_amd/csrc/mtm_context.hip
--- a/multitemplatematching-python_amd/csrc/mtm_context.hip
+++ b/multitemplatematching-python_amd/csrc/mtm_context.hip
@@ -315,6 +315,7 @@
     if (const char* v = std::getenv("MTM_SCREEN_L1")) c->screen_l1 = std::atoi(v);
     if (const char* v = std::getenv("MTM_TAIL_SCREEN")) c->tail_screen = std::atoi(v) != 0;
     if (const char* v = std::getenv("MTM_TAIL_SPLIT")) c->tail_split_force = std::max(0, std::atoi(v));
+    if (const char* v = std::getenv("MTM_TC_PACK")) c->tc_pack_on = std::atoi(v) != 0;
     if (const char* v = std::getenv("MTM_HOST_TRACE")) c->host_trace = std::atoi(v) != 0;
     if (const char* v = std::getenv("MTM_CLASS_LANES")) c->class_lanes = std::max(1, std::min(8, std::atoi(v)));
     if (const char* v = std::getenv("MTM_COMM_TIMEOUT_S")) c->comm_timeout_s = std::atof(v);
@@ -360,7 +361,7 @@
                       &c->mbf_maps, &c->f32_sq, &c->mbf_stats, &c->mbf_mu, &c->mbf_list, &c->mbf_best}) b->release();
     for (DevBuf* b : {&c->td, &c->tlist, &c->weights, &c->packs, &c->apacks, &c->maps, &c->hs1, &c->hs2, &c->stats, &c->hits,
                       &c->counters, &c->sched, &c->cands, &c->mask_td, &c->chash, &c->raw16, &c->stats_hi, &c->tsum, &c->stats_rsq, &c->stats_blk, &c->sq_planes, &c->comm_send,
-                      &c->comm_recv})
+                      &c->comm_recv, &c->tc_pack})
         b->release();
     if (c->pinned) (void)hipHostFree(c->pinned);
     if (c->pin_small) (void)hipHostFree(c->pin_small);
@@ -552,6 +553,21 @@
         r[9] = (size_t)k < c->tail_last.size() ? c->tail_last[(size_t)k] : 0;
         r[10] = (int32_t)sc.slabs.size();
         r[11] = sc.slab_nt;
+    }
+    return n;
+}
+
+int mtm_debug_tc_pack(mtm_ctx* c, int32_t* out, int cap_classes) {
+    if (!c || (!out && cap_classes > 0)) return MTM_E_INVALID;
+    MTM_NOT_IN_FLIGHT(c, "mtm_debug_tc_pack");
+    if (!c->placed) {
+        set_error("mtm_debug_tc_pack: no template set is placed (run a search first)");
+        return MTM_E_STATE;
+    }
+    const int n = (int)c->classes.size();
+    for (int k = 0; k < n && k < cap_classes; ++k) {
+        out[2 * k] = (size_t)k < c->tc_valid.size() ? c->tc_valid[(size_t)k] : 0;
+        out[2 * k + 1] = (size_t)k < c->tc_last.size() ? c->tc_last[(size_t)k] : 0;
     }
     return n;
 }
diff --git a/multitemplatematching-python_amd/csrc/mtm_ctx.h b/multitemplatematching-python_amd/csrc/mtm_ctx.h
--- a/multitemplatematching-python_amd/csrc/mtm_ctx.h
+++ b/multitemplatematching-python_amd/csrc/mtm_ctx.h
@@ -124,6 +124,7 @@
     long long mask_pack_off = -1;
     bool mask_bf16 = false;
     long long mbf_off_u = -1, mbf_off_v = -1, mbf_group_bytes = 0;
+    long long tcpack_off = -1;
     long long apack_off = 0;
     long long group_bytes = 0;
 };
@@ -173,6 +174,10 @@
     int tail_split_force = 0;
     std::vector<int> tail_valid;
     std::vector<int> tail_last;
+    int tc_pack_on = 1;
+    DevBuf tc_pack;
+    std::vector<int> tc_valid;
+    std::vector<int> tc_last;
     int f32_mfma = 1;
     int np1_backoff = 0, np1_backoff_len = 16;
     int seg_skip = 1;
@@ -389,6 +394,7 @@
 bool dot_variant_ok(int64_t v);
 int launch_stats(mtm_ctx* c, CallRoute& R, const SizeClass& sc, StatPlanes* out, int sb0 = 0, int sb1 = -1);
 int launch_tail_consts(mtm_ctx* c, const SizeClass& sc, int split, hipStream_t stream);
+int launch_tc_pack(mtm_ctx* c, const SizeClass& sc, hipStream_t stream);
 int launch_ncc(mtm_ctx* c, CallRoute& R, const SizeClass& sc, int list_off, int n_list, const StatPlanes& st, int only_li = -1,
                int yb0 = 0, int yb1 = -1);
 int ensure_maps(mtm_ctx* c);
diff --git a/multitemplatematching-python_amd/csrc/mtm_launch.hip b/multitemplatematching-python_amd/csrc/mtm_launch.hip
--- a/multitemplatematching-python_amd/csrc/mtm_launch.hip
+++ b/multitemplatematching-python_amd/csrc/mtm_launch.hip
@@ -111,9 +111,14 @@
     if (split <= 0 || sc.members.empty()) return MTM_OK;
     const bool mine = !c->classes.empty() && &sc >= c->classes.data() && &sc < c->classes.data() + c->classes.size();
     const size_t k = mine ? (size_t)(&sc - c->classes.data()) : 0;
-    if (mine && k < c->tail_valid.size() && c->tail_valid[k] == split) return MTM_OK;
-    MTMC(launch_tail_consts(c, sc, split, c->stream));
-    if (mine && k < c->tail_valid.size()) c->tail_valid[k] = split;
+    if (!(mine && k < c->tail_valid.size() && c->tail_valid[k] == split)) {
+        MTMC(launch_tail_consts(c, sc, split, c->stream));
+        if (mine && k < c->tail_valid.size()) c->tail_valid[k] = split;
+    }
+    if (mine && k < c->tc_valid.size() && c->tc_valid[k] != 0 && c->tc_valid[k] != 1 + split) {
+        MTMC(launch_tc_pack(c, sc, c->stream));
+        c->tc_valid[k] = 1 + split;
+    }
     return MTM_OK;
 }
 
@@ -778,9 +783,18 @@
     p.n_work = p.nseg * p.nyb * p.ntg;
     p.tail_split = (r2 && st.blkq != nullptr && only_li < 0 && !p.seg_skip) ? tail_split_for(c, R, sc) : 0;
     MTMC(ensure_tail_consts(c, sc, p.tail_split));
-    if (!c->classes.empty() && &sc >= c->classes.data() && &sc < c->classes.data() + c->classes.size() &&
-        (size_t)(&sc - c->classes.data()) < c->tail_last.size())
-        c->tail_last[(size_t)(&sc - c->classes.data())] = p.tail_split;
+    const bool mine = !c->classes.empty() && &sc >= c->classes.data() && &sc < c->classes.data() + c->classes.size();
+    const size_t cls_k = mine ? (size_t)(&sc - c->classes.data()) : 0;
+    if (mine && cls_k < c->tail_last.size()) c->tail_last[cls_k] = p.tail_split;
+    const bool tc_ok = c->tc_pack_on && r2 && mb == 2 && !R.ext && !R.sparse && only_li < 0 && c->chans == 1 && !sc.masked &&
+                       (c->method == MTM_TM_CCOEFF_NORMED || c->method == MTM_TM_CCORR_NORMED) && mine && sc.tcpack_off >= 0 &&
+                       cls_k < c->tc_valid.size() && c->tc_valid[cls_k] != 0 &&
+                       (p.tail_split == 0 || c->tc_valid[cls_k] == 1 + p.tail_split);
+    if (tc_ok) {
+        p.tc_on = 1;
+        p.tc_pack = c->tc_pack.as<uint8_t>() + sc.tcpack_off;
+    }
+    if (mine && cls_k < c->tc_last.size()) c->tc_last[cls_k] = tc_ok ? 1 : 0;
     const size_t stat_bytes = rm ? 0 : r2 ? (size_t)kMfRows * ((mb + 1) / 2) * 1024 + (p.tail_split ? mf_tail_lds_bytes() : 0)
                                           : (size_t)kMfRows * mf_stat_bytes_per_wave(c->chans == 3 ? 3 : 1);
     const bool ext = R.ext;
diff --git a/multitemplatematching-python_amd/csrc/mtm_mfma.hip.h b/multitemplatematching-python_amd/csrc/mtm_mfma.hip.h
--- a/multitemplatematching-python_amd/csrc/mtm_mfma.hip.h
+++ b/multitemplatematching-python_amd/csrc/mtm_mfma.hip.h
@@ -211,6 +211,26 @@
     else mfma_step<MB>(acc, qa, qb, a);
 }
 
+__device__ __forceinline__ void mf_stage_tile(const MfmaParams& p, uint8_t* smem, const uint8_t* grow, const int nchunk,
+                                              const int tid_i, const int wave, const int lane) {
+    typedef const __attribute__((address_space(1))) void* gptr_t;
+    typedef __attribute__((address_space(3))) void* lptr_t;
+    int ci = tid_i;
+    int r = (ci * p.cpr_magic) >> 16, d = ci - r * p.cpr;
+    uint8_t* lbase_w = smem + wave * 1024;
+    for (; ci - lane < nchunk; ci += 256) {
+        if (ci < nchunk)
+            __builtin_amdgcn_global_load_lds((gptr_t)(grow + (size_t)r * p.pitch + 16 * d), (lptr_t)lbase_w, 16, 0, 0);
+        lbase_w += 4096;
+        r += p.cpr_rstep;
+        d += p.cpr_dstep;
+        if (d >= p.cpr) {
+            d -= p.cpr;
+            ++r;
+        }
+    }
+}
+
 template <int MB, int METHOD, bool EXACT_DIV, bool MASKED = false, bool RM = false, int CH = 1, bool EXT = false,
           bool R2 = false, bool KP = false>
 __global__ __launch_bounds__(256, 2) void ncc_mfma_kernel(MfmaParams p, const TemplDev* __restrict__ td,
@@ -233,11 +253,16 @@
         clk0[0] = __builtin_readcyclecounter();
         clk0[1] = __builtin_amdgcn_s_memrealtime();
     }
+    constexpr bool kPack = R2 && !EXT && !MASKED && (METHOD == MTM_TM_CCORR_NORMED || METHOD == MTM_TM_CCOEFF_NORMED);
+#define MTM_TC_PACKED() (kPack && mf_opaque_sgpr(p.tc_on) != 0)
     const int per_xcd = (p.n_work + 7) >> 3;
     do {
     const int wid = (blockIdx.x & 7) * per_xcd + (blockIdx.x >> 3);
     if (wid >= p.n_work) break;
-    if (!EXT && METHOD != kMfRaw && p.hits_only) {
+    unsigned long long cand_n = 0ull;
+    if (MTM_TC_PACKED()) {
+        if (mf_opaque_sgpr(p.hits_only)) cand_n = __hip_atomic_load(p.cand_counter, __ATOMIC_RELAXED, __HIP_MEMORY_SCOPE_AGENT);
+    } else if (!EXT && METHOD != kMfRaw && p.hits_only) {
         if (threadIdx.x == 0)
             s_item[2] = __hip_atomic_load(p.cand_counter, __ATOMIC_RELAXED, __HIP_MEMORY_SCOPE_AGENT) > p.cand_cap ? 1 : 0;
         __syncthreads();
@@ -276,82 +301,82 @@
 
     MfTemplConst* tcl = reinterpret_cast<MfTemplConst*>(smem + p.tc_off);
     constexpr int kTGc = METHOD == kMfU16 ? 16 : kTG;
-    if (METHOD != kMfRaw && tid_i < (RM ? p.rm_nt : kTGc)) {
-        const int li = tg * kTGc + tid_i;
-        if (li < p.n_list) {
-            const TemplDev& T = td[tlist[li]];
+    if constexpr (kPack) {
+        if (!MTM_TC_PACKED() && tid_i < 16) {
+            const int li = tg * 16 + tid_i;
             MfTemplConst k;
-#pragma unroll
-            for (int cc = 0; cc < kMaxChans; ++cc) k.mean[cc] = T.mean[cc];
-            k.templ_norm = T.templ_norm;
-            k.templ_sum2 = T.templ_sum2;
-            k.mfma_k = T.mfma_k;
-            if constexpr (METHOD == kMfU16) {
-                const double kh = 128.0 * p.u16_tsum[li] - 16384.0 * p.u16_area;
-                const double kl = 128.0 * p.u16_tsum[p.u16_npad + li] - 16384.0 * p.u16_area;
-                k.mfma_k = 257.0 * (256.0 * kh + kl);
-            }
-            k.rtempl_norm = T.templ_norm > 0.0 ? 1.0 / T.templ_norm : 0.0;
-#pragma unroll
-            for (int cc = 0; cc < kMaxChans; ++cc) k.m128[cc] = 128.0 - T.mean[cc];
-            k.tms = T.templ2_mask2_sum;
-            k.rsqrt_tms = 1.0 / sqrt(T.templ2_mask2_sum);
-            k.map_off = T.map_off;
-            k.map_pitch = T.map_pitch;
-            k.all_ones = T.all_ones;
-            {
-                int ninf_hi = (int)0xfff00000;
-                asm volatile("" : "+v"(ninf_hi));
-                k.ext_thr_lo = __hiloint2double(ninf_hi, 0);
-            }
-            k.ext_hi = 0u;
-            k.flag_base = tlist[li] * p.flag_tstride;
-            if (EXT) {
-                const unsigned long long bk = __hip_atomic_load(&p.ext_best[2 * tlist[li] + p.cand_min], __ATOMIC_RELAXED,
-                                                                __HIP_MEMORY_SCOPE_AGENT);
-                if (bk) {
-                    const uint32_t hiw = (uint32_t)(bk >> 32);
-                    const double sc = (double)mf_order_float(p.cand_min ? ~hiw : hiw);
-                    const double ql = p.cand_min ? -sc : sc;
-                    k.ext_hi = hiw;
-                    k.ext_thr_lo = ql - 1e-6 * fmax(1.0, fabs(ql));
-                }
-            }
+            if (li < p.n_list) mf_templ_const(k, td[tlist[li]], tlist[li], p.flag_tstride);
+            else mf_templ_const_none(k);
             tcl[tid_i] = k;
-        } else if (!RM) {
-            MfTemplConst k;
-#pragma unroll
-            for (int cc = 0; cc < kMaxChans; ++cc) k.mean[cc] = 0.0, k.m128[cc] = 0.0;
-            k.templ_norm = 1.0;
-            k.templ_sum2 = 0.0;
-            k.mfma_k = -1e300;
-            k.rtempl_norm = 0.0;
-            k.tms = 1.0;
-            k.rsqrt_tms = 0.0;
-            k.map_off = 0;
-            k.map_pitch = 0;
-            k.all_ones = 0;
-            k.ext_thr_lo = 1e300;
-            k.ext_hi = 0xFFFFFFFFu;
-            k.flag_base = 0;
-            tcl[tid_i] = k;
-        }
-    }
-
-    if constexpr (R2 && !EXT && (METHOD == MTM_TM_CCORR_NORMED || METHOD == MTM_TM_CCOEFF_NORMED)) {
-        if (mf_opaque_sgpr(p.tail_split) > 0 && tid_i < 16) {
-            MfTailConst* ttl = reinterpret_cast<MfTailConst*>(smem + p.st_off + kMfRows * ((MB + 1) / 2) * 1024 + kMfTailRecBytes);
-            const int li = tg * 16 + tid_i;
-            MfTailConst k;
+            if (mf_opaque_sgpr(p.tail_split) > 0) {
+                MfTailConst* ttl = reinterpret_cast<MfTailConst*>(smem + p.st_off + kMfRows * ((MB + 1) / 2) * 1024 + kMfTailRecBytes);
+                MfTailConst u;
+                if (li < p.n_list) mf_tail_const(u, td[tlist[li]]);
+                else mf_tail_const_none(u);
+                ttl[tid_i] = u;
+            }
+        }
+    } else {
+        if (METHOD != kMfRaw && tid_i < (RM ? p.rm_nt : kTGc)) {
+            const int li = tg * kTGc + tid_i;
             if (li < p.n_list) {
                 const TemplDev& T = td[tlist[li]];
-#pragma unroll
-                for (int r = 0; r < 2; ++r) k.k[r] = T.tail_k[r], k.d[r] = T.tail_d[r], k.g[r] = T.tail_g[r];
-            } else {
-#pragma unroll
-                for (int r = 0; r < 2; ++r) k.k[r] = -1e300, k.d[r] = 0.0, k.g[r] = 0.0;
-            }
-            ttl[tid_i] = k;
+                MfTemplConst k;
+#pragma unroll
+                for (int cc = 0; cc < kMaxChans; ++cc) k.mean[cc] = T.mean[cc];
+                k.templ_norm = T.templ_norm;
+                k.templ_sum2 = T.templ_sum2;
+                k.mfma_k = T.mfma_k;
+                if constexpr (METHOD == kMfU16) {
+                    const double kh = 128.0 * p.u16_tsum[li] - 16384.0 * p.u16_area;
+                    const double kl = 128.0 * p.u16_tsum[p.u16_npad + li] - 16384.0 * p.u16_area;
+                    k.mfma_k = 257.0 * (256.0 * kh + kl);
+                }
+                k.rtempl_norm = T.templ_norm > 0.0 ? 1.0 / T.templ_norm : 0.0;
+#pragma unroll
+                for (int cc = 0; cc < kMaxChans; ++cc) k.m128[cc] = 128.0 - T.mean[cc];
+                k.tms = T.templ2_mask2_sum;
+                k.rsqrt_tms = 1.0 / sqrt(T.templ2_mask2_sum);
+                k.map_off = T.map_off;
+                k.map_pitch = T.map_pitch;
+                k.all_ones = T.all_ones;
+                {
+                    int ninf_hi = (int)0xfff00000;
+                    asm volatile("" : "+v"(ninf_hi));
+                    k.ext_thr_lo = __hiloint2double(ninf_hi, 0);
+                }
+                k.ext_hi = 0u;
+                k.flag_base = tlist[li] * p.flag_tstride;
+                if (EXT) {
+                    const unsigned long long bk = __hip_atomic_load(&p.ext_best[2 * tlist[li] + p.cand_min], __ATOMIC_RELAXED,
+                                                                    __HIP_MEMORY_SCOPE_AGENT);
+                    if (bk) {
+                        const uint32_t hiw = (uint32_t)(bk >> 32);
+                        const double sc = (double)mf_order_float(p.cand_min ? ~hiw : hiw);
+                        const double ql = p.cand_min ? -sc : sc;
+                        k.ext_hi = hiw;
+                        k.ext_thr_lo = ql - 1e-6 * fmax(1.0, fabs(ql));
+                    }
+                }
+                tcl[tid_i] = k;
+            } else if (!RM) {
+                MfTemplConst k;
+#pragma unroll
+                for (int cc = 0; cc < kMaxChans; ++cc) k.mean[cc] = 0.0, k.m128[cc] = 0.0;
+                k.templ_norm = 1.0;
+                k.templ_sum2 = 0.0;
+                k.mfma_k = -1e300;
+                k.rtempl_norm = 0.0;
+                k.tms = 1.0;
+                k.rsqrt_tms = 0.0;
+                k.map_off = 0;
+                k.map_pitch = 0;
+                k.all_ones = 0;
+                k.ext_thr_lo = 1e300;
+                k.ext_hi = 0xFFFFFFFFu;
+                k.flag_base = 0;
+                tcl[tid_i] = k;
+            }
         }
     }
 
@@ -399,6 +424,29 @@
 
     const uint8_t* apack_g = apack + slab_ap + (long long)tg * (R2 ? 1 : MB) * p.group_bytes + (size_t)lane * 16;
     bool tail_out = false;
+    v4i a_first = v4i{0, 0, 0, 0};
+    if constexpr (kPack) {
+        if (MTM_TC_PACKED()) {
+            typedef const __attribute__((address_space(1))) void* gptr_t;
+            typedef __attribute__((address_space(3))) void* lptr_t;
+            const uint8_t* tcg = p.tc_pack + (size_t)tg * kMfTcGroupBytes + (size_t)lane * 16;
+            if (wave < 3) {
+                if (wave * 1024 + lane * 16 < kMfTcTemplBytes)
+                    __builtin_amdgcn_global_load_lds((gptr_t)(tcg + wave * 1024), (lptr_t)(smem + p.tc_off + wave * 1024), 16, 0, 0);
+            } else if (mf_opaque_sgpr(p.tail_split) > 0 && lane * 16 < kMfTcGroupBytes - kMfTcTemplBytes) {
+                __builtin_amdgcn_global_load_lds((gptr_t)(tcg + kMfTcTemplBytes),
+                                                 (lptr_t)(smem + p.st_off + kMfRows * ((MB + 1) / 2) * 1024 + kMfTailRecBytes), 16, 0, 0);
+            }
+            const int krows0 = min(kMfChunkR2, p.h + MB - 1);
+            mf_stage_tile(p, smem, p.img + (size_t)y0 * p.pitch + x0, (krows0 + (kMfRows - 1) * wave_rows) * p.cpr, tid_i, wave, lane);
+            a_first = *reinterpret_cast<const v4i*>(apack_g);
+            asm volatile("s_waitcnt vmcnt(0)" : "+v"(cand_n) : : "memory");
+            const int hits_only = mf_opaque_sgpr(p.hits_only);
+            if (hits_only && tid_i == 0) s_item[2] = cand_n > p.cand_cap ? 1 : 0;
+            __syncthreads();
+            if (hits_only && s_item[2]) break;
+        }
+    }
 
     for (int c = 0; c < p.chans; ++c) {
         const uint8_t* plane = p.img + slab_img + c * p.plane;
@@ -426,6 +474,7 @@
         v4i r2_prev = v4i{0, 0, 0, 0};
         for (int cy0 = 0; cy0 < krows; cy0 += kChunk) {
             const int ch = min(kChunk, krows - cy0);
+            if (!(MTM_TC_PACKED() && cy0 == 0)) {
             __syncthreads();
             {
                 typedef const __attribute__((address_space(1))) void* gptr_t;
@@ -450,6 +499,7 @@
                 asm volatile("s_waitcnt vmcnt(0)" ::: "memory");
             }
             __syncthreads();
+            }
             if constexpr (R2) {
                 const uint8_t* aptr = apack_g + (size_t)cy0 * 1024;
                 const uint8_t* lbase = smem + wave * wave_rows * p.lds_pitch + (j + q) * 16;
@@ -485,7 +535,13 @@
                 MTM_R2_STEP(qx, qy, aC, aB, qx2, qy2, aA)                   \
                 MTM_R2_STEP(qx2, qy2, aA, aC, qx, qy, aB)                   \
                 MTM_R2_STEP(qx, qy, aB, aA, qx2, qy2, aC)
-                MTM_R2_LOAD(qx, qy, aA)
+                if (MTM_TC_PACKED() && cy0 == 0) {
+                    qx = *reinterpret_cast<const v4i*>(lbase + loff);
+                    qy = *reinterpret_cast<const v4i*>(lbase + loff + 16);
+                    aA = a_first;
+                } else {
+                    MTM_R2_LOAD(qx, qy, aA)
+                }
                 int ks = 0;
                 const int split = (!EXT && kNormed) ? mf_opaque_sgpr(p.tail_split) : 0;
                 if (split > 0) {
@@ -1632,6 +1688,7 @@
         const unsigned long long dt = __builtin_readcyclecounter() - clk0[0], dr = __builtin_amdgcn_s_memrealtime() - clk0[1];
         if (dr > 0) *p.clk_out = (float)((double)dt * 100.0 / (double)dr);
     }
+#undef MTM_TC_PACKED
 }
 
 }
diff --git a/multitemplatematching-python_amd/csrc/mtm_mfma_params.h b/multitemplatematching-python_amd/csrc/mtm_mfma_params.h
--- a/multitemplatematching-python_amd/csrc/mtm_mfma_params.h
+++ b/multitemplatematching-python_amd/csrc/mtm_mfma_params.h
@@ -45,7 +45,9 @@
     int only_li;
     int tc_off;
     int st_off;
-    int pad0_[4];
+    int tc_on;
+    const uint8_t* tc_pack;
+    int pad0_;
     mtm_hit* cand_hits;
     unsigned long long* cand_counter;
     unsigned long long cand_cap;
@@ -107,8 +109,57 @@
 struct MfTailConst {
     double k[2], d[2], g[2];
 };
+__device__ __forceinline__ void mf_templ_const(MfTemplConst& k, const TemplDev& T, int templ, int flag_tstride) {
+#pragma unroll
+    for (int cc = 0; cc < kMaxChans; ++cc) k.mean[cc] = T.mean[cc];
+    k.templ_norm = T.templ_norm;
+    k.templ_sum2 = T.templ_sum2;
+    k.mfma_k = T.mfma_k;
+    k.rtempl_norm = T.templ_norm > 0.0 ? 1.0 / T.templ_norm : 0.0;
+#pragma unroll
+    for (int cc = 0; cc < kMaxChans; ++cc) k.m128[cc] = 128.0 - T.mean[cc];
+    k.tms = T.templ2_mask2_sum;
+    k.rsqrt_tms = 1.0 / sqrt(T.templ2_mask2_sum);
+    k.map_off = T.map_off;
+    k.map_pitch = T.map_pitch;
+    k.all_ones = T.all_ones;
+    {
+        int ninf_hi = (int)0xfff00000;
+        asm volatile("" : "+v"(ninf_hi));
+        k.ext_thr_lo = __hiloint2double(ninf_hi, 0);
+    }
+    k.ext_hi = 0u;
+    k.flag_base = templ * flag_tstride;
+}
+__device__ __forceinline__ void mf_templ_const_none(MfTemplConst& k) {
+#pragma unroll
+    for (int cc = 0; cc < kMaxChans; ++cc) k.mean[cc] = 0.0, k.m128[cc] = 0.0;
+    k.templ_norm = 1.0;
+    k.templ_sum2 = 0.0;
+    k.mfma_k = -1e300;
+    k.rtempl_norm = 0.0;
+    k.tms = 1.0;
+    k.rsqrt_tms = 0.0;
+    k.map_off = 0;
+    k.map_pitch = 0;
+    k.all_ones = 0;
+    k.ext_thr_lo = 1e300;
+    k.ext_hi = 0xFFFFFFFFu;
+    k.flag_base = 0;
+}
+__device__ __forceinline__ void mf_tail_const(MfTailConst& k, const TemplDev& T) {
+#pragma unroll
+    for (int r = 0; r < 2; ++r) k.k[r] = T.tail_k[r], k.d[r] = T.tail_d[r], k.g[r] = T.tail_g[r];
+}
+__device__ __forceinline__ void mf_tail_const_none(MfTailConst& k) {
+#pragma unroll
+    for (int r = 0; r < 2; ++r) k.k[r] = -1e300, k.d[r] = 0.0, k.g[r] = 0.0;
+}
 constexpr int kMfTailRecBytes = kMfRows * 1024;
 constexpr int mf_tail_lds_bytes() { return kMfTailRecBytes + 16 * (int)sizeof(MfTailConst); }
+constexpr int kMfTcTemplBytes = 16 * (int)sizeof(MfTemplConst);
+constexpr int kMfTcGroupBytes = kMfTcTemplBytes + 16 * (int)sizeof(MfTailConst);
+static_assert(kMfTcTemplBytes == 2304 && kMfTcGroupBytes == 3072, "one LDS-DMA instruction per wave (mtm_mfma.hip.h)");
 
 using MfmaFn = void (*)(MfmaParams, const TemplDev*, const int*, const uint8_t*, StatPlanes, float*);
 
diff --git a/multitemplatematching-python_amd/csrc/mtm_placement.hip b/multitemplatematching-python_amd/csrc/mtm_placement.hip
--- a/multitemplatematching-python_amd/csrc/mtm_placement.hip
+++ b/multitemplatematching-python_amd/csrc/mtm_placement.hip
@@ -437,6 +437,14 @@
     return MTM_OK;
 }
 
+int queue_tc_pack(mtm_ctx* c, const SizeClass& sc, hipStream_t stream) {
+    const int n = (int)sc.members.size();
+    hipLaunchKernelGGL(tc_pack_kernel, dim3((unsigned)((n + 15) / 16)), dim3(64), 0, stream, c->td.as<TemplDev>(),
+                       c->tlist.as<int>() + sc.tlist_off, n, c->tc_pack.as<uint8_t>() + sc.tcpack_off);
+    HIPC(hipGetLastError());
+    return MTM_OK;
+}
+
 size_t place_apacks(const mtm_ctx* c, SizeClass& sc, Bump& a, Bump& ts) {
     const int n_cls = (int)sc.members.size(), groups = mfma_groups_alloc(n_cls);
     size_t bytes = 0;
@@ -684,6 +692,18 @@
     for (const SizeClass& sc : P.classes)
         if (sc.tail_split > 0 && sc.kernel == MTM_KERNEL_MFMA && !sc.members.empty())
             MTMC(queue_tail_consts(c, sc, sc.tail_split, c->stream));
+    {
+        size_t tc_bytes = 0;
+        for (SizeClass& sc : P.classes) {
+            sc.tcpack_off = -1;
+            if (!c->tc_pack_on || sc.r2 != 2 || sc.kernel != MTM_KERNEL_MFMA || sc.members.empty()) continue;
+            sc.tcpack_off = (long long)tc_bytes;
+            tc_bytes += (sc.members.size() + 15) / 16 * (size_t)mtm::kMfTcGroupBytes;
+        }
+        if (tc_bytes) MTMC(c->tc_pack.ensure(tc_bytes));
+        for (const SizeClass& sc : P.classes)
+            if (sc.tcpack_off >= 0) MTMC(queue_tc_pack(c, sc, c->stream));
+    }
     const bool local_sources = P.any_host_pack || P.any_mbf || w_off || p_off || ts_off || new_units;
     if (local_sources) HIPC(hipStreamSynchronize(c->stream));
     c->place_pending = !local_sources;
@@ -692,9 +712,12 @@
     c->classes.swap(P.classes);
     c->tail_valid.assign(c->classes.size(), 0);
     c->tail_last.assign(c->classes.size(), 0);
+    c->tc_valid.assign(c->classes.size(), 0);
+    c->tc_last.assign(c->classes.size(), 0);
     for (size_t k = 0; k < c->classes.size(); ++k) {
         const SizeClass& sc = c->classes[k];
         if (sc.tail_split > 0 && sc.kernel == MTM_KERNEL_MFMA && !sc.members.empty()) c->tail_valid[k] = sc.tail_split;
+        if (sc.tcpack_off >= 0) c->tc_valid[k] = 1 + c->tail_valid[k];
     }
     c->td_host.swap(P.td);
     c->tlist_host.swap(P.tlist);
@@ -710,6 +733,7 @@
 namespace mtmi {
 
 int launch_tail_consts(mtm_ctx* c, const SizeClass& sc, int split, hipStream_t stream) { return queue_tail_consts(c, sc, split, stream); }
+int launch_tc_pack(mtm_ctx* c, const SizeClass& sc, hipStream_t stream) { return queue_tc_pack(c, sc, stream); }
 
 int place_templates(mtm_ctx* c) {
     if (!c->have_image || !c->have_templ) {
diff --git a/multitemplatematching-python_amd/csrc/mtm_templates.hip.h b/multitemplatematching-python_amd/csrc/mtm_templates.hip.h
--- a/multitemplatematching-python_amd/csrc/mtm_templates.hip.h
+++ b/multitemplatematching-python_amd/csrc/mtm_templates.hip.h
@@ -3,6 +3,7 @@
 #include <cstdint>
 
 #include "mtm_kernels.h"
+#include "mtm_mfma_params.h"
 #include "mtm_templates_params.h"
 
 namespace mtm {
@@ -197,4 +198,23 @@
     t.tail_g[r] = gg;
 }
 
-}
+__global__ __launch_bounds__(64) void tc_pack_kernel(const TemplDev* __restrict__ td, const int* __restrict__ tl, int n_list,
+                                                     uint8_t* __restrict__ out) {
+    const int i = threadIdx.x, li = blockIdx.x * 16 + i;
+    if (i >= 16) return;
+    uint8_t* g = out + (size_t)blockIdx.x * kMfTcGroupBytes;
+    MfTemplConst k;
+    MfTailConst u;
+    if (li < n_list) {
+        const TemplDev& T = td[tl[li]];
+        mf_templ_const(k, T, tl[li], 0);
+        mf_tail_const(u, T);
+    } else {
+        mf_templ_const_none(k);
+        mf_tail_const_none(u);
+    }
+    reinterpret_cast<MfTemplConst*>(g)[i] = k;
+    reinterpret_cast<MfTailConst*>(g + kMfTcTemplBytes)[i] = u;
+}
+
+}
```
